# Jackson-D-Taylor/PINT

Hardware: AMD Instinct MI355X
Metric: GLS fits/sec, 68-PSR x 10k-TOA synthetic PTA (whole node) (higher is better)
Workload: dtype f64+dd; 1 GPU; pta68x10k GLSFitter.fit_toas(maxiter=1) incl. noise realisations (the 68-pulsar PTA, LPT-sharded over 1 rank(s)); npsr=68, ntoas=10000, K_cols_max=178, launch=direct, pipelines=2, parallelism=pulsar shards x1 (LPT, no data-path collective)

## Files before the change

include/pint_amd.h:

```cpp
#ifndef PINT_AMD_H
#define PINT_AMD_H

#include <stddef.h>
#include <stdint.h>

#ifdef __cplusplus
extern "C" {
#endif

#define PINT_OK 0
#define PINT_E_INVALID 1
#define PINT_E_HIP 2
#define PINT_E_NOT_PD 3
#define PINT_E_KEPLER 4
#define PINT_E_PARAM 5
#define PINT_E_SIGMA 6

#define PINT_MAX_COLS 320
#define PINT_MAX_F 16
#define PINT_MAX_DMK 10
#define PINT_MAX_FD 10
#define PINT_MAX_JUMP 64
#define PINT_MAX_GLITCH 64
#define PINT_MAX_WAVEX 128
// ... 100 lines not shown
    int32_t col_toff[PINT_MAX_COLS];
} pint_spec_t;

typedef struct pint_ctx pint_ctx;

pint_ctx *pint_ctx_create(int device);
void pint_ctx_destroy(pint_ctx *ctx);
const char *pint_last_error(pint_ctx *ctx);

void pint_release_cache(void);
int pint_device_count(void);
int pint_nslot(void);

int pint_add_pulsar(pint_ctx *ctx, const pint_toas_t *toas, const pint_spec_t *spec,
                    const double *red_freq, const double *red_phi);
int pint_add_pulsar_cols(pint_ctx *ctx, const pint_toa_cols_t *cols, const pint_spec_t *spec,
                         const double *red_freq, const double *red_phi);
int pint_set_wavex(pint_ctx *ctx, int psr, int o_wx, int nwx, int o_dmwx, int ndmwx);
int pint_set_chromatic(pint_ctx *ctx, int psr, int o_cm, int ncm, int o_cmwx, int ncmwx);

int pint_set_instances(pint_ctx *ctx, int ninst, const int32_t *inst_psr, const double *tables);

int pint_set_grid(pint_ctx *ctx, int psr, int npts, const double *base, int nvar, const int32_t *var_toff,
                  const int64_t *var_stride, const int64_t *var_size, const double *vals, int64_t k0);
int pint_get_tables(pint_ctx *ctx, double *tables_out);
int pint_set_tables(pint_ctx *ctx, const double *tables);

int pint_eval(pint_ctx *ctx, int want_M);

int pint_read_resids(pint_ctx *ctx, double *time_resid, double *phase_resid, double *chi2_wls);
int pint_read_eval(pint_ctx *ctx, double *phase_hi, double *phase_lo, double *ftaylor, double *delay);
int pint_read_designmatrix(pint_ctx *ctx, double *M);

int pint_fit_step(pint_ctx *ctx, int mode);
int pint_read_step(pint_ctx *ctx, double *dpars, double *errs, double *cov, double *chi2_lin);

int pint_apply_step(pint_ctx *ctx, const double *lambda_);
int pint_apply_step_uniform(pint_ctx *ctx, double lambda_);
int pint_fit_step_apply(pint_ctx *ctx, int mode, double lambda_);

int pint_save_tables(pint_ctx *ctx);
int pint_restore_tables(pint_ctx *ctx);

int pint_chi2_gls(pint_ctx *ctx, double *chi2);

int pint_chi2_wls(pint_ctx *ctx, double *chi2);

int pint_set_ecorr(pint_ctx *ctx, int psr, int nep, const int32_t *ep_ptr, const int32_t *ep_idx,
                   const double *ep_phi);

int pint_fit_layout(pint_ctx *ctx, int psr, int32_t *out4);
int pint_vgram_layout(pint_ctx *ctx, int psr, int32_t *out4);
int pint_set_wideband(pint_ctx *ctx, int psr, const double *pp_dm, const double *pp_dme,
                      const double *dm_sigma, const uint64_t *dmjump_mask);
int pint_dm_resids(pint_ctx *ctx, int subtract_mean, int use_weighted_mean, double *resid_out,
                   double *chi2_out);

int pint_set_lazy(pint_ctx *ctx, int lazy);
int pint_check(pint_ctx *ctx);

#ifndef PINT_NSLOT
#define PINT_NSLOT 4
#endif
int pint_step_end(pint_ctx *ctx, int *slot);
int pint_fit_step_enqueue(pint_ctx *ctx, int restore, int mode, double lambda_, double *dpars, double *errs,
                          double *cov, double *chi2lin, double *noise_red, double *noise_ecorr, double *noise_dm,
                          double *chi2, int *slot);
int pint_check_step(pint_ctx *ctx, int slot);
#define PINT_OPT_BLOCKED_SOLVE 1
#define PINT_OPT_VGRAM 2
#define PINT_OPT_TIMING_MASK 3
#define PINT_OPT_TIMING_EVERY 8
#define PINT_OPT_REFINE 4
#define PINT_OPT_VBIN 5
#define PINT_OPT_WBFIT 6
#define PINT_OPT_COV_DEFER 7
#define PINT_OPT_SCHUR 9
#define PINT_OPT_SMALL 10
#define PINT_OPT_LA_CHOL 11
#define PINT_OPT_EFUSE 12
#define PINT_OPT_LANE_SOLVE 13
#define PINT_OPT_SPIN_EVAL 14
#define PINT_OPT_SOLVE_W8 15
int pint_set_option(pint_ctx *ctx, int key, int value);
#define PINT_EIG_MAXDEG 8
int pint_solve_eig(pint_ctx *ctx, int mode, const double *threshold, int32_t *ndeg, double *degvec,
                   int degstride);

int pint_lognorm(pint_ctx *ctx, int gls, double *out);

int pint_capture_begin(pint_ctx *ctx);
int pint_capture_end(pint_ctx *ctx);
int pint_graph_launch(pint_ctx *ctx);
#define PINT_QUERY_NVGRAM 1
#define PINT_QUERY_NSPLIT 2
#define PINT_QUERY_NSPINEVAL 3
int pint_query(pint_ctx *ctx, int key);
void *pint_host_alloc(size_t bytes);
void pint_host_free(void *p);
int pint_debug_read(pint_ctx *ctx, int which, double *out);
int pint_debug_gram(pint_ctx *ctx, int pre_ecorr, double *out);
int pint_debug_set_resids(pint_ctx *ctx, const double *time_resid);

int pint_read_norms(pint_ctx *ctx, int mode, double *out);

int pint_inst_status(pint_ctx *ctx, int32_t *out);

int pint_noise_resids(pint_ctx *ctx, double *red, double *ecorr);
int pint_noise_resids_dm(pint_ctx *ctx, double *dm);

int pint_last_timing(pint_ctx *ctx, double *ms8);
int pint_sync(pint_ctx *ctx);

int pint_set_resids(pint_ctx *ctx, const double *time_resid);
int pint_set_sigma(pint_ctx *ctx, int psr, const double *sigma_s);
int pint_set_noise_weights(pint_ctx *ctx, int psr, const double *red_phi, const double *ep_phi);
int pint_set_noise_classes(pint_ctx *ctx, int psr, int ncls, const int32_t *cls_ptr, const int32_t *cls_idx,
                           const double *sigma0_us);
int pint_noise_lnlike(pint_ctx *ctx, const int32_t *kind, const double *cls_qf, const double *ep_w, double *out3,
                      double *cls_g, double *ep_g);

#ifdef __cplusplus
}
#endif
#endif
```

pint_amd/csrc/physics.hpp:

```cpp
#pragma once
#include "dd.hpp"
#include "../../include/pint_amd.h"

namespace pint {

constexpr double C_KMS = 299792.458;
constexpr double AU_KM = 149597870.7;
constexpr double KPC_KM = 3.0856775814913674e16;
constexpr double TSUN = 4.92549094830932e-06;
__device__ __constant__ const double TPLANET[5] = {TSUN / 1047.3486, TSUN / 3497.898, TSUN / 408523.71, TSUN / 22902.98,
                               TSUN / 19412.24};
constexpr double DMCONST = 4149.377593360996;
constexpr double DAYSEC = 86400.0;
constexpr double DJY = 365.25;
constexpr double ERFA_DC = 173.1446326742403;
constexpr double DR2AS = 206264.80624709636;
constexpr double MAS_RAD = 4.84813681109536e-09;
constexpr double HA_RAD = 0.2617993877991494;
constexpr double DEG_RAD = 0.017453292519943295;
constexpr double MASYR_RADS = 1.5362818500441604e-16;
constexpr double YR_S = 31557600.0;
constexpr double TWO_PI = 6.283185307179586;
constexpr double PI_D = 3.141592653589793;
constexpr double INV_C_KMS = 1.0 / C_KMS;
constexpr double INV_AU_KM = 1.0 / AU_KM;
constexpr double INV_AUC = 1.0 / (AU_KM * C_KMS);
constexpr double INV_KPC_KM = 1.0 / KPC_KM;
constexpr double INV_DJY = 1.0 / DJY;
constexpr double INV_TWO_PI = 1.0 / TWO_PI;
constexpr int NINV = 64;
__device__ __constant__ const double INV_HI[NINV] = {0.0, 1.0, 0.5, 0.3333333333333333, 0.25, 0.2, 0.16666666666666666, 0.14285714285714285, 0.125, 0.1111111111111111, 0.1, 0.09090909090909091, 0.08333333333333333, 0.07692307692307693, 0.07142857142857142, 0.06666666666666667, 0.0625, 0.058823529411764705, 0.05555555555555555, 0.05263157894736842, 0.05, 0.047619047619047616, 0.045454545454545456, 0.043478260869565216, 0.041666666666666664, 0.04, 0.038461538461538464, 0.037037037037037035, 0.03571428571428571, 0.034482758620689655, 0.03333333333333333, 0.03225806451612903, 0.03125, 0.030303030303030304, 0.029411764705882353, 0.02857142857142857, 0.027777777777777776, 0.02702702702702703, 0.02631578947368421, 0.02564102564102564, 0.025, 0.024390243902439025, 0.023809523809523808, 0.023255813953488372, 0.022727272727272728, 0.022222222222222223, 0.021739130434782608, 0.02127659574468085, 0.020833333333333332, 0.02040816326530612, 0.02, 0.0196078431372549, 0.019230769230769232, 0.018867924528301886, 0.018518518518518517, 0.01818181818181818, 0.017857142857142856, 0.017543859649122806, 0.017241379310344827, 0.01694915254237288, 0.016666666666666666, 0.01639344262295082, 0.016129032258064516, 0.015873015873015872};
__device__ __constant__ const double INV_LO[NINV] = {0.0, 0.0, 0.0, 1.850371707708594e-17, 0.0, -1.1102230246251566e-17, 9.25185853854297e-18, 7.93016446160826e-18, 0.0, 6.1679056923619804e-18, -5.551115123125783e-18, -2.523234146875356e-18, 4.625929269271485e-18, -4.270088556250602e-18, 3.96508223080413e-18, 9.251858538542971e-19, 0.0, 8.163404592832033e-19, 3.0839528461809902e-18, 2.921639538487254e-18, -2.7755575615628915e-18, 2.64338815386942e-18, -1.261617073437678e-18, 1.206764157201257e-18, 2.3129646346357427e-18, -8.326672684688674e-19, -2.135044278125301e-18, 2.05596856412066e-18, 1.982541115402065e-18, 4.785444071660157e-19, 4.625929269271486e-19, 8.953411488912552e-19, 0.0, -8.410780489584519e-19, 4.0817022964160166e-19, 8.921435019309293e-19, 1.5419764230904951e-18, -1.50030138462859e-18, 1.460819769243627e-18, 8.896017825522087e-19, -1.3877787807814458e-18, -8.46206573647223e-19, 1.32169407693471e-18, 3.2273925134452225e-19, -6.30808536718839e-19, -8.480870326997723e-19, 6.033820786006285e-19, 5.167261417803255e-19, 1.1564823173178713e-18, 1.6285159162231251e-18, -4.163336342344337e-19, 2.7211348642773444e-19, -1.0675221390626506e-18, 7.20073895688486e-19, 1.02798428206033e-18, 8.831319514063744e-19, 9.912705577010326e-19, 9.73879846162418e-19, 2.3927220358300787e-19, 5.880418562633244e-20, 2.312964634635743e-19, -8.531426931033477e-19, 4.476705744456276e-19, 8.8112938462314e-19};
PD double inv_int(int k) { return k < NINV ? INV_HI[k] : 1.0 / (double)k; }
PD dd dd_div_int(dd a, int k) { return k < NINV ? dd_mul(a, dd_make(INV_HI[k], INV_LO[k])) : dd_div_d(a, (double)k); }

PD double pval(const double* P, int o) { return P[o] + P[o + 1]; }
PD dd pdd(const double* P, int o) { return dd_make(P[o], P[o + 1]); }

struct PmState {
    double p[3], v1[3], tl1;
};

struct PmTrig {
    double cra, sra, cdec, sdec, cra2, sra2, cdec2, sdec2;
};

PD void pm_setup_trig(double pmr, double pmd, double px, const PmTrig& T, PmState& st);

PD void pm_setup(double ra, double dec, double pmr, double pmd, double px, PmState& st) {
    const double ra2 = ra + pmr, dec2 = dec + pmd;
    const PmTrig T = {cos(ra), sin(ra), cos(dec), sin(dec), cos(ra2), sin(ra2), cos(dec2), sin(dec2)};
    pm_setup_trig(pmr, pmd, px, T, st);
}

PD void pm_setup_trig(double pmr, double pmd, double px, const PmTrig& T, PmState& st) {
    double a1[3] = {T.cra * T.cdec, T.sra * T.cdec, T.sdec};
    double b1[3] = {T.cra2 * T.cdec2, T.sra2 * T.cdec2, T.sdec2};
    double cx = a1[1] * b1[2] - a1[2] * b1[1];
    double cy = a1[2] * b1[0] - a1[0] * b1[2];
    double cz = a1[0] * b1[1] - a1[1] * b1[0];
    double ss = sqrt(cx * cx + cy * cy + cz * cz);
    double cs = a1[0] * b1[0] + a1[1] * b1[1] + a1[2] * b1[2];
    double px1a = px;
    if ((ss != 0.0 || cs != 0.0) && !(cs > 0.0 && 326.0 * (ss / cs) * (1.0 + 1e-12) < px1a)) {
        const double pm = 326.0 * atan2(ss, cs);
        if (px1a < pm) px1a = pm;
    }
    if (px1a < 5e-7) px1a = 5e-7;
    double w = px1a >= 1e-7 ? px1a : 1e-7;
    double r = DR2AS / w;
    double rad = pmr / DJY, decd = pmd / DJY;
    double st_ = T.sra, ct = T.cra, sp = T.sdec, cp = T.cdec;
    double rcp = r * cp;
    double x = rcp * ct, y = rcp * st_;
    double rpd = r * decd;
    double ww = rpd * sp;
    double p[3] = {x, y, r * sp};
    double v[3] = {-y * rad - ww * ct, x * rad - ww * st_, rpd * cp};
    double vm = sqrt(v[0] * v[0] + v[1] * v[1] + v[2] * v[2]);
    if (vm / ERFA_DC > 0.5) { v[0] = v[1] = v[2] = 0.0; }
    double pm_ = sqrt(p[0] * p[0] + p[1] * p[1] + p[2] * p[2]);
    double xu[3] = {p[0] / pm_, p[1] / pm_, p[2] / pm_};
    double vsr = xu[0] * v[0] + xu[1] * v[1] + xu[2] * v[2];
    double usr[3] = {vsr * xu[0], vsr * xu[1], vsr * xu[2]};
    double ust[3] = {v[0] - usr[0], v[1] - usr[1], v[2] - usr[2]};
    double vst = sqrt(ust[0] * ust[0] + ust[1] * ust[1] + ust[2] * ust[2]);
    double betsr = vsr / ERFA_DC, betst = vst / ERFA_DC;
    double bett = betst, betr = betsr, d = 1.0, del = 0.0, od = 0.0, odel = 0.0, odd = 0.0, oddel = 0.0;
    for (int i = 0; i < 100; i++) {
        d = 1.0 + betr;
        double w2 = betr * betr + bett * bett;
        del = -w2 / (sqrt(1.0 - w2) + 1.0);
        betr = d * betsr + del;
        bett = d * betst;
        if (i > 0) {
            double dd_ = fabs(d - od), ddel = fabs(del - odel);
            if (i > 1 && dd_ >= odd && ddel >= oddel) break;
            odd = dd_;
            oddel = ddel;
        }
        od = d;
        odel = del;
    }
    double wr = (betsr != 0.0) ? d + del / betsr : 1.0;
    for (int k = 0; k < 3; k++) {
        st.p[k] = p[k];
        st.v1[k] = wr * usr[k] + d * ust[k];
    }
    st.tl1 = pm_ / ERFA_DC;
}

PD void pm_dir(const PmState& st, double dt_days, double out[3]) {
    const double* p = st.p;
    const double* v1 = st.v1;
    const double tl1 = st.tl1;
    double q[3] = {p[0] + (dt_days + tl1) * v1[0], p[1] + (dt_days + tl1) * v1[1], p[2] + (dt_days + tl1) * v1[2]};
    double r2 = q[0] * q[0] + q[1] * q[1] + q[2] * q[2];
// ... 765 lines not shown
}

PD double bt_deriv(const BinState& B, int pid) {
    const double e = B.ecc, sE = B.sinE, cE = B.cosE, tt0 = B.tt0, a1 = B.a1;
    const double sw = B.sw, cw = B.cw, sq = B.sqE, iom = B.iomeE;
    const double iP = B.iPBs, iP2 = iP * iP;
    const double dL1_dE = -a1 * sw * sE;
    const double dL2_dE = (a1 * cw * sq + B.GAMMA) * cE;
    const double dE_dECC = sE * iom;
    double dL1 = 0.0, dL2 = 0.0, dE = 0.0;
    switch (pid) {
        case PINT_B_A1: case PINT_B_A1DOT: {
            const double f = (pid == PINT_B_A1DOT) ? tt0 : 1.0;
            dL1 = f * sw * (cE - e);
            dL2 = f * cw * sq * sE;
        } break;
        case PINT_B_OM: case PINT_B_OMDOT: {
            const double f = (pid == PINT_B_OMDOT) ? tt0 : 1.0;
            dL1 = f * a1 * cw * (cE - e);
            dL2 = -f * a1 * sw * sq * sE;
        } break;
        case PINT_B_ECC: case PINT_B_EDOT: {
            const double f = (pid == PINT_B_EDOT) ? tt0 : 1.0;
            dL1 = f * (a1 * sw + dL1_dE * dE_dECC);
            dL2 = f * (-a1 * cw * e * sE / sq + dL2_dE * dE_dECC);
        } break;
        case PINT_B_GAMMA: dL2 = sE; break;
        case PINT_B_T0:
            dE = (((B.PBDOT - B.XPBDOT) * tt0 * iP - 1.0) * TWO_PI * iP - B.EDOT * sE) * iom;
            break;
        case PINT_B_PB: dE = TWO_PI * ((B.PBDOT + B.XPBDOT) * tt0 * tt0 * iP2 * iP - tt0 * iP2) * iom; break;
        case PINT_B_PBDOT: case PINT_B_XPBDOT: dE = -PI_D * tt0 * tt0 * iP2 * iom; break;
        default: break;
    }
    if (dE != 0.0) {
        dL1 = dL1_dE * dE;
        dL2 = dL2_dE * dE;
    }
    return B.R0 * (dL1 + dL2);
}

struct ToaRow {
    dd tdb;
    double freq;
    double pos[3], vel[3], sun[3];
    const double* planet;
    uint32_t flags;
    uint64_t jmask;
    int dmx_a, dmx_b;
    const int32_t* dmx_x;
    int dmx_x0, dmx_x1;
};

struct EvalOut {
    dd phase;
    double delay;
    double fdt;
    double ftaylor;
    double dmc;
    double inv_f2;
    int status;
};

PD dd spin_phase(const pint_spec_t& S, const double* P, dd dt) {
    int m = S.nf;
    dd r = pdd(P, S.o_F + 2 * (m - 1));
    for (int j = m - 1; j >= 1; j--) {
        r = dd_add(dd_div_int(dd_mul(r, dt), j + 1), pdd(P, S.o_F + 2 * (j - 1)));
    }
    return dd_mul(r, dt);
}
PD double spin_freq(const pint_spec_t& S, const double* P, double dt) {
    int m = S.nf;
    double r = pval(P, S.o_F + 2 * (m - 1));
    for (int j = m - 1; j >= 1; j--) r = r * dt * inv_int(j) + pval(P, S.o_F + 2 * (j - 1));
    return r;
}

struct ColRun {
    int kind, col0, cnt, idx0;
    int dcol0;
    int pad_[3];
};

struct EvalHead {
    double delay;
    double gLON, gLAT, gPMLON, gPMLAT, gPX;
    double inv_f2, dt_yr_dm, logf;
    double swg;
};
constexpr int EVAL_HEAD_W = 10;

struct EvalSpin {
    dd dt;
    double dtd, chain;
};
PD void eval_spin_a(const pint_spec_t& S, const double* P, const InstConst& C, const ToaRow& t, double delay,
                    EvalOut& o, EvalSpin& sp) {
    o.delay = delay;
    dd dt0 = dd_mul_d(dd_sub(t.tdb, pdd(P, S.o_PEPOCH)), DAYSEC);
    sp.dt = dd_add_d(dt0, -delay);
    sp.dtd = dd_to_d(sp.dt);
    o.fdt = spin_freq(S, P, sp.dtd);
    o.ftaylor = spin_freq(S, P, dd_to_d(dt0));
    sp.chain = o.fdt * C.iF0;
}

PD double glitch_dt(const pint_spec_t& S, const double* P, dd tdb, double delay, int k) {
    const int o = S.o_GLITCH + 2 * PINT_GL_NPAR * k;
    return dd_to_d(dd_add_d(dd_mul_d(dd_sub(tdb, pdd(P, o + 2 * PINT_GL_EP)), DAYSEC), -delay));
}
PD double glitch_phase_at(const double* G, double dt) {
    double ph = pval(G, 2 * PINT_GL_PH) +
                dt * (pval(G, 2 * PINT_GL_F0) +
                      dt * (0.5 * pval(G, 2 * PINT_GL_F1) + dt * ((1.0 / 6.0) * pval(G, 2 * PINT_GL_F2))));
    const double f0d = pval(G, 2 * PINT_GL_F0D);
    if (f0d != 0.0) {
        const double tau = pval(G, 2 * PINT_GL_TD) * DAYSEC;
        ph += f0d * tau * (1.0 - exp(-dt / tau));
    }
    return ph;
}
PD double glitch_col_at(const double* G, int which, double dt, double iF0) {
    const double tau = pval(G, 2 * PINT_GL_TD) * DAYSEC;
    const double f0d = pval(G, 2 * PINT_GL_F0D);
    const double e = tau != 0.0 ? exp(-dt / tau) : 0.0;
    double d;
    switch (which) {
        case PINT_GL_PH: d = 1.0; break;
        case PINT_GL_F0: d = dt; break;
        case PINT_GL_F1: d = 0.5 * dt * dt; break;
        case PINT_GL_F2: d = (1.0 / 6.0) * dt * dt * dt; break;
        case PINT_GL_F0D: d = tau * (1.0 - e); break;
        case PINT_GL_TD:
            d = tau != 0.0 ? (f0d * (1.0 - e) - f0d * e * (dt / tau)) * DAYSEC : 0.0;
            break;
        default:
            d = -(pval(G, 2 * PINT_GL_F0) +
                  dt * (pval(G, 2 * PINT_GL_F1) + 0.5 * dt * pval(G, 2 * PINT_GL_F2)) + f0d * e) * DAYSEC;
    }
    return -d * iF0;
}

PD dd glitch_row_phase(const pint_spec_t& S, const double* P, dd tdb, double delay, dd ph) {
    for (int k = 0; k < S.nglitch; k++) {
        const double gdt = glitch_dt(S, P, tdb, delay, k);
        if (gdt > 0.0) ph = dd_add_d(ph, glitch_phase_at(P + S.o_GLITCH + 2 * PINT_GL_NPAR * k, gdt));
    }
    return ph;
}
PD void glitch_row_columns(const pint_spec_t& S, const double* P, dd tdb, double delay, double iF0, double* Mb,
                           unsigned r, long ld, const ColRun* runs, int nrun, bool compact) {
    for (int u = 0; u < nrun; u++) {
        const ColRun R = runs[u];
        if (R.kind != PINT_COL_GLITCH) continue;
        double* colp = Mb + (long)(compact ? R.dcol0 : R.col0) * ld;
        for (int j = 0; j < R.cnt; j++, colp += ld) {
            const int k = (R.idx0 + j) / PINT_GL_NPAR, which = (R.idx0 + j) - PINT_GL_NPAR * k;
            const double gdt = glitch_dt(S, P, tdb, delay, k);
            colp[r] = gdt > 0.0 ? glitch_col_at(P + S.o_GLITCH + 2 * PINT_GL_NPAR * k, which, gdt, iF0) : 0.0;
        }
    }
}

template <int BIN>
PD void eval_spin_b(const pint_spec_t& S, const double* P, const InstConst& C, const ToaRow& t, const EvalHead& h,
                    const EvalSpin& sp, EvalOut& o, double* Mb, unsigned r, long ld, const ColRun* runs, int nrun,
                    bool compact, const double* swg = nullptr) {
    const double chain = sp.chain, dtd = sp.dtd;
    dd ph = spin_phase(S, P, sp.dt);
    if (S.njump > 0 && t.jmask) {
        dd F0 = pdd(P, S.o_F);
        for (int k = 0; k < S.njump; k++)
            if ((t.jmask >> k) & 1ull) ph = dd_add(ph, dd_mul(dd_make(pval(P, S.o_JUMP + 2 * k)), F0));
    }
    if (S.o_PHOFF >= 0 && r < (unsigned)ld) ph = dd_sub(ph, pdd(P, S.o_PHOFF));
    o.phase = ph;
    if (!Mb) return;
    const double iF0 = C.iF0;
    const double dt_yr_dm = h.dt_yr_dm, logf = h.logf;
    const double gLON = h.gLON * chain;
    const double gLAT = h.gLAT * chain;
    const double gPMLON = h.gPMLON * chain;
    const double gPMLAT = h.gPMLAT * chain;
    const double gPX = h.gPX * chain;
    const double dmc = chain * DMCONST * h.inv_f2;
    o.dmc = dmc;
    for (int u = 0; u < nrun; u++) {
        const ColRun R = runs[u];
        if (compact && R.kind == PINT_COL_DMX) continue;
        double* colp = Mb + (long)(compact ? R.dcol0 : R.col0) * ld;
        switch (R.kind) {
            case PINT_COL_OFFSET: colp[r] = iF0; break;
            case PINT_COL_F: {
                double v = 1.0;
                for (int j = 1; j <= R.idx0; j++) v = v * dtd * inv_int(j);
                for (int j = 0; j < R.cnt; j++, colp += ld) {
                    v = v * dtd * inv_int(R.idx0 + j + 1);
                    colp[r] = -v * iF0;
                }
            } break;
            case PINT_COL_JUMP:
                for (int j = 0; j < R.cnt; j++, colp += ld) colp[r] = ((t.jmask >> (R.idx0 + j)) & 1ull) ? -1.0 : 0.0;
                break;
            case PINT_COL_LON: colp[r] = gLON; break;
            case PINT_COL_LAT: colp[r] = gLAT; break;
            case PINT_COL_PMLON: colp[r] = gPMLON; break;
            case PINT_COL_PMLAT: colp[r] = gPMLAT; break;
            case PINT_COL_PX: colp[r] = gPX; break;
            case PINT_COL_DM: {
                double v = 1.0;
                for (int j = 1; j <= R.idx0; j++) v = v * dt_yr_dm * inv_int(j);
                for (int j = 0; j < R.cnt; j++, colp += ld) {
                    if (j > 0) v = v * dt_yr_dm * inv_int(R.idx0 + j);
                    colp[r] = dmc * v;
                }
            } break;
            case PINT_COL_NESW: {
                double g = h.swg;
                if (swg) {
                    unsigned rr = r;
                    asm volatile("" : "+v"(rr));
                    g = swg[rr];
                }
                colp[r] = h.inv_f2 > 1.0 ? 0.0 : dmc * g;
            } break;
            case PINT_COL_DMX:
                for (int j = 0; j < R.cnt; j++, colp += ld) {
                    const int idx = R.idx0 + j;
                    bool in = t.dmx_a == idx || t.dmx_b == idx;
                    for (int k = t.dmx_x0; k < t.dmx_x1; k++) in |= t.dmx_x[k] == idx;
                    colp[r] = in ? dmc : 0.0;
                }
                break;
            case PINT_COL_FD: {
                double v = 1.0;
                for (int j = 0; j <= R.idx0; j++) v *= logf;
                for (int j = 0; j < R.cnt; j++, colp += ld) {
                    if (j > 0) v *= logf;
                    colp[r] = chain * v;
                }
            } break;
            case PINT_COL_BIN:
                if (BIN == 0)
                    for (int j = 0; j < R.cnt; j++, colp += ld) colp[r] = 0.0;
                break;
            default:
                for (int j = 0; j < R.cnt; j++, colp += ld) colp[r] = 0.0;
        }
    }
}

struct EvalPre {
    EvalHead h;
    double fd;
    double L[3];
};
PD void eval_pre(const pint_spec_t& S, const double* P, const InstConst& C, const ToaRow& t, EvalOut& o, bool wantM,
                 EvalPre& pre, const double* swg, unsigned r) {
    o.status = 0;
    o.dmc = 0.0;
    double delay = 0.0;
    double L[3] = {0, 0, 1};
    double tdb_f = dd_to_d(t.tdb);
    bool has_pos = (t.flags & 2u) != 0;
    bool is_bary = (t.flags & 1u) != 0;
    double rr = 0.0, re_dot_L = 0.0;
    double px_mas = S.o_px >= 0 ? pval(P, S.o_px) : 0.0;
    if (S.astrometry) {
        psr_dir_icrs(C, tdb_f, L);
        rr = t.pos[0] * t.pos[0] + t.pos[1] * t.pos[1] + t.pos[2] * t.pos[2];
        re_dot_L = t.pos[0] * L[0] + t.pos[1] * L[1] + t.pos[2] * L[2];
        if (has_pos) {
            double d = -re_dot_L * INV_C_KMS;
            if (px_mas != 0.0) {
                d += (0.5 * (rr * px_mas * INV_KPC_KM) * (1.0 - re_dot_L * re_dot_L / rr)) * INV_C_KMS;
            }
            delay += d;
        }
    }
    if (S.shapiro && !is_bary) {
        double rs = sqrt(t.sun[0] * t.sun[0] + t.sun[1] * t.sun[1] + t.sun[2] * t.sun[2]);
        double rct = t.sun[0] * L[0] + t.sun[1] * L[1] + t.sun[2] * L[2];
        double ds = -2.0 * TSUN * log((rs - rct) * INV_AU_KM);
        if (S.shapiro == 2) {
#pragma unroll 1
            for (int q = 0; q < 5; q++) {
                const double x = t.planet[3 * q], y = t.planet[3 * q + 1], z = t.planet[3 * q + 2];
                const double rp = sqrt(x * x + y * y + z * z);
                const double rcp = x * L[0] + y * L[1] + z * L[2];
                ds += -2.0 * TPLANET[q] * log((rp - rcp) * INV_AU_KM);
            }
        }
        delay += ds;
    }
    double bfreq = t.freq;
    if (S.astrometry) {
        double vdl = t.vel[0] * L[0] + t.vel[1] * L[1] + t.vel[2] * L[2];
        bfreq = t.freq * (1.0 - vdl * INV_C_KMS);
    }
    double inv_f2 = 1.0 / (bfreq * bfreq);
    o.inv_f2 = inv_f2;
    if (S.o_NE_SW >= 0) delay += (pval(P, S.o_NE_SW) * swg[r]) * DMCONST * inv_f2;
    double dt_yr_dm = 0.0;
    if (S.ndm > 0) {
        bool any = false;
        for (int k = 1; k < S.ndm; k++) any |= (pval(P, S.o_DM + 2 * k) != 0.0);
        if (S.o_DMEPOCH >= 0) {
            dd dtd = dd_sub(t.tdb, pdd(P, S.o_DMEPOCH));
            dt_yr_dm = dd_to_d(dtd) * INV_DJY;
        }
        double x = any ? dt_yr_dm : 0.0;
        double dm = pval(P, S.o_DM + 2 * (S.ndm - 1));
        for (int k = S.ndm - 1; k >= 1; k--) dm = dm * x * inv_int(k) + pval(P, S.o_DM + 2 * (k - 1));
        delay += dm * DMCONST * inv_f2;
    }
    if (S.ndmx > 0) {
        double dmx = 0.0;
        if (t.dmx_a >= 0) dmx += pval(P, S.o_DMX + 2 * t.dmx_a);
        if (t.dmx_b >= 0) dmx += pval(P, S.o_DMX + 2 * t.dmx_b);
        for (int k = t.dmx_x0; k < t.dmx_x1; k++) dmx += pval(P, S.o_DMX + 2 * t.dmx_x[k]);
        delay += dmx * DMCONST * inv_f2;
    }
    double logf = 0.0;
    double fd = 0.0;
    if (S.nfd > 0) {
        logf = log(bfreq * 1e-3);
        if (!isfinite(logf)) logf = 0.0;
        for (int k = S.nfd; k >= 1; k--) fd = fd * logf + pval(P, S.o_FD + 2 * (k - 1));
        fd *= logf;
    }
    double gLON = 0, gLAT = 0, gPMLON = 0, gPMLAT = 0, gPX = 0;
    if (wantM && S.astrometry) {
        double u[3] = {t.pos[0], t.pos[1], t.pos[2]};
        if (S.astrometry == 2) {
            double ue[3] = {u[0], u[1], u[2]};
            icrs_to_ecl(S.obliquity, ue, u);
        }
        const double r_km = sqrt(rr);
        const double ir = r_km > 0.0 ? 1.0 / r_km : 0.0;
        const double ced_sdl = (C.splon * u[0] - C.cplon * u[1]) * ir;
        const double ced_cdl = (C.cplon * u[0] + C.splon * u[1]) * ir;
        const double sed = u[2] * ir;
        const double te_s = S.o_POSEPOCH >= 0 ? dd_to_d(dd_mul_d(dd_sub(t.tdb, pdd(P, S.o_POSEPOCH)), DAYSEC)) : 0.0;
        const double rc = r_km * INV_C_KMS;
        gLON = rc * (ced_sdl * C.cplat) * (S.astrometry == 1 ? HA_RAD : DEG_RAD);
        gLAT = rc * (ced_cdl * C.splat - sed * C.cplat) * DEG_RAD;
        gPMLON = rc * ced_sdl * te_s * MASYR_RADS;
        gPMLAT = rc * (ced_cdl * C.splat - C.cplat * sed) * te_s * MASYR_RADS;
        gPX = 0.5 * ((rr - re_dot_L * re_dot_L) * INV_AUC) * MAS_RAD;
    }
    pre.h = {delay, gLON, gLAT, gPMLON, gPMLAT, gPX, inv_f2, dt_yr_dm, logf, 0.0};
    pre.fd = fd;
    pre.L[0] = L[0];
    pre.L[1] = L[1];
    pre.L[2] = L[2];
}

PD void eval_head(const pint_spec_t& S, const double* P, const InstConst& C, const ToaRow& t, EvalHead& h,
                  const double* swg, unsigned r) {
    EvalOut o;
    EvalPre pre;
    eval_pre(S, P, C, t, o, true, pre, swg, r);
    h = pre.h;
    if (S.o_NE_SW >= 0) h.swg = swg[r];
    if (S.nfd > 0) h.delay += pre.fd;
}

template <int BIN>
PD void eval_toa(const pint_spec_t& S, const double* P, const InstConst& C, const ToaRow& t, EvalOut& o,
                 double* Mb, unsigned r, long ld, const ColRun* runs, int nrun, bool compact, const double* swg) {
    EvalPre pre;
    eval_pre(S, P, C, t, o, Mb != nullptr, pre, swg, r);
    double delay = pre.h.delay;
    const double* L = pre.L;
    const double fd = pre.fd;
    const double inv_f2 = pre.h.inv_f2, dt_yr_dm = pre.h.dt_yr_dm, logf = pre.h.logf;
    const double gLON = pre.h.gLON, gLAT = pre.h.gLAT, gPMLON = pre.h.gPMLON, gPMLAT = pre.h.gPMLAT, gPX = pre.h.gPX;
    BinState B;
    B.status = 0;
    if (BIN == 1 || BIN == 3) {
        ell1_setup<BIN == 3>(S, P, C, t.tdb, delay, B);
        delay += B.delay;
    } else if (BIN == 2) {
        ddm_setup(S, P, C, t.tdb, delay, B);
        delay += B.delay;
        if (B.status) o.status = B.status;
    } else if (BIN == 4) {
        bt_setup(S, P, C, t.tdb, delay, B);
        delay += B.delay;
        if (B.status) o.status = B.status;
    } else if (BIN == 5) {
        double ko[3] = {t.pos[0], t.pos[1], t.pos[2]}, kp[3] = {L[0], L[1], L[2]};
        if (S.astrometry == 2) {
            icrs_to_ecl(S.obliquity, t.pos, ko);
            icrs_to_ecl(S.obliquity, L, kp);
        }
        ddm_setup<true>(S, P, C, t.tdb, delay, B, ko, kp);
        delay += B.delay;
        if (B.status) o.status = B.status;
    }
    if (S.nfd > 0) delay += fd;
    EvalSpin sp;
    eval_spin_a(S, P, C, t, delay, o, sp);
    const double chain = sp.chain;
    if (Mb && BIN != 0) {
        Ell1Grad eg;
        if (BIN == 1 || BIN == 3) ell1_grad<BIN == 3>(B, eg);
        for (int u = 0; u < nrun; u++) {
            const ColRun R = runs[u];
            if (R.kind != PINT_COL_BIN) continue;
            double* colp = Mb + (long)(compact ? R.dcol0 : R.col0) * ld;
            for (int j = 0; j < R.cnt; j++, colp += ld) {
                const int pid = S.col_index[R.col0 + j];
                double d = 0.0;
                if (BIN == 1 || BIN == 3) d = ell1_deriv(B, eg, pid);
                if (BIN == 2) d = ddm_deriv(B, pid);
                if (BIN == 4) d = bt_deriv(B, pid);
                if (BIN == 5) d = ddm_deriv<true>(B, pid);
                colp[r] = chain * d * bin_unit_factor(pid);
            }
        }
    }
    const EvalHead h = {delay, gLON, gLAT, gPMLON, gPMLAT, gPX, inv_f2, dt_yr_dm, logf, 0.0};
    eval_spin_b<BIN>(S, P, C, t, h, sp, o, Mb, r, ld, runs, nrun, compact, S.o_NE_SW >= 0 ? swg : nullptr);
}

}
```

pint_amd/csrc/pint_hip.hip:

```cpp
#include <hip/hip_runtime.h>
#include <hip/hip_ext.h>
#include <string>
#include <vector>
#include <cstring>
#include <cstdio>
#include <algorithm>
#include <cmath>
#include <cstdlib>
#include <map>
#include <type_traits>
#include <mutex>
#include <functional>
#include <chrono>
#include "physics.hpp"

using namespace pint;

typedef double double4_t __attribute__((ext_vector_type(4)));

__device__ __forceinline__ void rot(double& c, double& s, double c1, double s1) {
    const double cn = c * c1 - s * s1;
    s = s * c1 + c * s1;
    c = cn;
}
// ... 254 lines not shown
    __shared__ InstConst sC;
    inst_setup_wave(*reinterpret_cast<const pint_spec_t*>(sS), staged ? sP : Pg, sC, sx, threadIdx.x);
    __syncthreads();
    if (threadIdx.x == 0) *out = sC;
}

constexpr int PREP_LANE_TAB = 64;
__global__ __launch_bounds__(64) void k_prep_lanes(const PsrDev* __restrict__ psrs, const InstDev* __restrict__ insts,
                                                   int ninst, double* __restrict__ tables,
                                                   const double* __restrict__ tables0, InstConst* __restrict__ ic) {
    const int q = blockIdx.x * 64 + threadIdx.x;
    if (q >= ninst) return;
    const InstDev I = insts[q];
    const pint_spec_t& S = *psrs[I.psr].spec;
    const double* P = tables + I.toff;
    if (tables0) {
        const int ts = S.tstride;
        for (int i = 0; i < ts; i++) tables[I.toff + i] = tables0[I.toff + i];
        P = tables0 + I.toff;
    }
    InstConst C;
    inst_setup_seq(S, P, C);
    ic[q] = C;
}
__global__ __launch_bounds__(64) void k_apply_lanes(const PsrDev* __restrict__ psrs, const InstDev* __restrict__ insts,
                                                    int ninst, double* __restrict__ tables,
                                                    const double* __restrict__ dpars, const double* __restrict__ lam,
                                                    InstConst* __restrict__ ic, double lam_u) {
    const int q = blockIdx.x * 64 + threadIdx.x;
    if (q >= ninst) return;
    const InstDev I = insts[q];
    const pint_spec_t& S = *psrs[I.psr].spec;
    double* P = tables + I.toff;
    const double li = lam ? lam[q] : lam_u;
    if (li != 0.0) {
        for (int c = 0; c < S.ncol; c++) {
            const int o = S.col_toff[c];
            if (o < 0) continue;
            const dd v = dd_add_d(dd_make(P[o], P[o + 1]), li * dpars[I.coff + c]);
            P[o] = v.hi;
            P[o + 1] = v.lo;
        }
    }
    InstConst C;
    inst_setup_seq(S, P, C);
    ic[q] = C;
}

__global__ __launch_bounds__(PREP_T) void k_prep(const PsrDev* __restrict__ psrs, const InstDev* __restrict__ insts,
                                                 double* __restrict__ tables, const double* __restrict__ tables0,
                                                 InstConst* __restrict__ ic) {
    const InstDev I = insts[blockIdx.x];
    const PsrDev& Pd = psrs[I.psr];
    const int ts = Pd.spec->tstride;
    if (tables0) {
        for (int i = threadIdx.x; i < ts; i += PREP_T) tables[I.toff + i] = tables0[I.toff + i];
        prep_one(Pd.spec, tables0 + I.toff, ts, ic + blockIdx.x);
        return;
    }
    prep_one(Pd.spec, tables + I.toff, ts, ic + blockIdx.x);
}

constexpr int EVAL_MAXTAB = 512;
constexpr int EVAL_MAXRUN = 64;
struct alignas(16) EvalLds {
    pint_spec_t S;
    InstConst C;
    ColRun R[EVAL_MAXRUN];
    double P[EVAL_MAXTAB];
    double X[4];
    double red[8];
};
constexpr int EF_ROWS = 254;

struct EvalRestore {
    double* tables;
    InstConst* ic;
    double* rph;
    double* epart;
    const double* swg;
};

__device__ __forceinline__ void load_toa_row(const PsrDev& Pd, const pint_spec_t& S, unsigned r, ToaRow& t) {
    t.tdb = dd_make(Pd.tdb_hi[r], Pd.tdb_lo[r]);
    t.freq = Pd.freq[r];
#pragma unroll
    for (int k = 0; k < 3; k++) {
        t.pos[k] = Pd.pos[3 * r + k];
        t.vel[k] = Pd.vel[3 * r + k];
        t.sun[k] = Pd.sun[3 * r + k];
    }
    t.planet = S.shapiro == 2 ? Pd.planet + 15 * r : nullptr;
    t.flags = Pd.flags[r];
    t.jmask = Pd.jmask[r];
    t.dmx_a = Pd.dmx_a[r];
    t.dmx_b = Pd.dmx_b[r];
    t.dmx_x = Pd.dmx_x;
    t.dmx_x0 = Pd.dmx_x ? Pd.dmx_x[r] : 0;
    t.dmx_x1 = Pd.dmx_x ? Pd.dmx_x[r + 1] : 0;
}

template <int WANT_M, int BIN>
__device__ __forceinline__ void eval_row(const pint_spec_t& S, EvalLds& L, const PsrDev& Pd, const InstDev& I, bool stP,
                                         bool stR, int nrun, const double* __restrict__ tables, unsigned r, int n,
                                         bool own, double* __restrict__ Mout, double* __restrict__ dmxv, int compact,
                                         int write_red, int* __restrict__ status, int* __restrict__ istatus, int ii,
                                         double* __restrict__ ph_hi, double* __restrict__ ph_lo,
                                         double* __restrict__ ftay, double* __restrict__ delay_out,
                                         double* __restrict__ dfac, const double* __restrict__ swg, EvalOut& o) {
    const double* P = stP ? L.P : tables + I.toff;
    ToaRow t;
    load_toa_row(Pd, S, r, t);
    double* Mb = WANT_M ? (Mout + I.moff) : nullptr;
    const bool rowM = WANT_M && own && r < (unsigned)n;
    const bool cmp = WANT_M && compact && Pd.dsplit;
    eval_toa<BIN>(S, P, L.C, t, o, rowM ? Mb : nullptr, r, n, stR ? L.R : Pd.runs, nrun, cmp, swg ? swg + I.roff : nullptr);
    if (!own) return;
    if (rowM && cmp) dmxv[I.ooff + r] = o.dmc;
    if (o.status) {
        atomicOr(status, 1 << o.status);
        atomicOr(istatus + ii, 1 << o.status);
    }
    ph_hi[I.roff + r] = o.phase.hi;
    ph_lo[I.roff + r] = o.phase.lo;
    ftay[I.roff + r] = o.ftaylor;
    delay_out[I.roff + r] = o.delay;
    const bool dmn = S.dmn0 < S.nred;
    const double Dfac = 1400.0 * 1400.0 * o.inv_f2;
    if (WANT_M && rowM && dmn) dfac[I.ooff + r] = Dfac;
    if (WANT_M && rowM && S.nred > 0 && (write_red || dmn) && !(cmp && Pd.vg)) {
        dd ts = dd_mul_d(t.tdb, DAYSEC);
        double* colp = Mb + (long)(cmp ? Pd.red0c : S.ncol) * n;
        for (int k = write_red ? 0 : S.dmn0; k < S.nred; k++) {
            dd x = dd_mul(ts, dd_make(Pd.red_freq[k], Pd.red_freq[S.nred + k]));
            double fr = dd_to_d(dd_sub(x, dd_floor(x)));
            double sn, cs;
            sincos(TWO_PI * fr, &sn, &cs);
            const double sc = k >= S.dmn0 ? Dfac : 1.0;
            colp[2L * k * n + r] = sn * sc;
            colp[2L * k * n + r + n] = cs * sc;
        }
    }
}

template <int WANT_M, int BIN>
__device__ __forceinline__ void eval_block(int b, const PsrDev* __restrict__ psrs, const InstDev* __restrict__ insts,
                                           const int* __restrict__ blk_inst, const int* __restrict__ blk_row0,
                                           const double* __restrict__ tables, const InstConst* __restrict__ ic,
                                           double* __restrict__ ph_hi, double* __restrict__ ph_lo,
                                           double* __restrict__ ftay, double* __restrict__ delay_out,
                                           double* __restrict__ Mout, double* __restrict__ dmxv, int compact,
                                           int write_red, int* __restrict__ status, int* __restrict__ istatus,
                                           double* __restrict__ dfac, EvalLds& L, EvalRestore rs) {
    int ii = blk_inst[b];
    const InstDev I = insts[ii];
    const PsrDev& Pd = psrs[I.psr];
    const int ts = I.ts, nrun = I.nrun;
    const bool stP = ts <= EVAL_MAXTAB, stR = nrun <= EVAL_MAXRUN;
    {
        static_assert(sizeof(pint_spec_t) % 16 == 0 && sizeof(InstConst) % 16 == 0 && sizeof(ColRun) % 16 == 0,
                      "eval staging: 16-byte words");
        constexpr int NS = (int)(sizeof(pint_spec_t) / 16), NC = (int)(sizeof(InstConst) / 16);
        constexpr int RW = (int)(sizeof(ColRun) / 16);
        static_assert(NS <= 512 && NC + EVAL_MAXRUN * RW <= 256 && EVAL_MAXTAB <= 512, "eval staging: two rounds of 256");
        const int t = threadIdx.x;
        const int NR = stR ? nrun * RW : 0;
        const uint4* sg = reinterpret_cast<const uint4*>(I.spec);
        const uint4* cg = reinterpret_cast<const uint4*>(ic + ii);
        const uint4* rg = reinterpret_cast<const uint4*>(I.runs);
        const double* pg = tables + I.toff;
        const bool hs0 = t < NS, hs1 = t + 256 < NS, hc = t < NC, hr = !hc && t < NC + NR;
        const bool hp0 = stP && t < ts, hp1 = stP && t + 256 < ts;
        uint4 s0 = {}, s1 = {}, cr = {};
        double p0 = 0.0, p1 = 0.0;
        if (hs0) s0 = sg[t];
        if (hs1) s1 = sg[t + 256];
        if (hc) cr = cg[t];
        else if (hr) cr = rg[t - NC];
        if (hp0) p0 = pg[t];
        if (hp1) p1 = pg[t + 256];
        uint4* sd = reinterpret_cast<uint4*>(&L.S);
        if (hs0) sd[t] = s0;
        if (hs1) sd[t + 256] = s1;
        if (hc) reinterpret_cast<uint4*>(&L.C)[t] = cr;
        else if (hr) reinterpret_cast<uint4*>(L.R)[t - NC] = cr;
        if (hp0) L.P[t] = p0;
        if (hp1) L.P[t + 256] = p1;
    }
    __syncthreads();
    wgp_stamp(0, true);
    if (rs.tables && blk_row0[b] == 0) {
        for (int k = threadIdx.x; k < ts; k += blockDim.x) rs.tables[I.toff + k] = stP ? L.P[k] : tables[I.toff + k];
        const int* cs = reinterpret_cast<const int*>(&L.C);
        int* cd = reinterpret_cast<int*>(rs.ic + ii);
        for (int k = threadIdx.x; k < (int)(sizeof(InstConst) / 4); k += blockDim.x) cd[k] = cs[k];
    }
    const pint_spec_t& S = L.S;
    const int n = I.n;
    const bool ef = rs.epart != nullptr;
    const int lt = threadIdx.x;
    unsigned r;
    bool own;
    if (ef) {
        r = lt < EF_ROWS ? (unsigned)(blk_row0[b] + lt) : (lt == EF_ROWS ? 0u : (unsigned)n);
        own = lt < EF_ROWS ? r < (unsigned)n : (lt == EF_ROWS + 1 && blk_row0[b] == 0);
        if (lt < EF_ROWS && r >= (unsigned)n) r = 0;
    } else {
        r = (unsigned)(blk_row0[b] + lt);
        own = r <= (unsigned)n;
        if (!own) return;
    }
    EvalOut o;
    eval_row<WANT_M, BIN>(S, L, Pd, I, stP, stR, nrun, tables, r, n, own, Mout, dmxv, compact, write_red, status, istatus,
                          ii, ph_hi, ph_lo, ftay, delay_out, dfac, rs.swg, o);
    wgp_stamp(1, false);
    if (!ef) return;
    if (lt == EF_ROWS) {
        L.X[2] = o.phase.hi;
        L.X[3] = o.phase.lo;
    } else if (lt == EF_ROWS + 1) {
        L.X[0] = o.phase.hi;
        L.X[1] = o.phase.lo;
    }
    __syncthreads();
    const dd tz = dd_make(L.X[0], L.X[1]);
    dd d0 = dd_make(0.0);
    if (!S.track_pn && S.subtract_mean) d0 = dd_add_d(dd_sub(dd_make(L.X[2], L.X[3]), tz), Pd.dpn[0]);
    double sw = 0.0, swx = 0.0;
    if (lt < EF_ROWS && own) {
        const dd d = dd_add_d(dd_sub(dd_make(o.phase.hi, o.phase.lo), tz), Pd.dpn[r]);
        double full;
        if (S.track_pn) {
            full = dd_to_d(dd_add_d(d, -Pd.pn[r]));
        } else {
            const dd x = dd_sub(d, d0);
            full = dd_to_d(dd_sub(x, dd_round_half_up(x)));
        }
        rs.rph[I.roff - ii + r] = full;
        const double lw = Pd.isig[r];
        const double w = S.weighted_mean ? lw * lw : 1.0;
        sw += w;
        swx += w * full;
    }
    if (S.subtract_mean) {
        double v[2] = {swx, sw};
        block_sums<4, 2>(v, L.red);
        if (lt == 0) {
            const long eb = I.eb0 + blk_row0[b] / EF_ROWS;
            rs.epart[2 * eb] = v[1];
            rs.epart[2 * eb + 1] = v[0];
        }
    }
}

__device__ __forceinline__ double sw_geometry_row(const PsrDev& Pd, const InstConst& C, int i) {
    double L[3];
    psr_dir_icrs(C, dd_to_d(dd_make(Pd.tdb_hi[i], Pd.tdb_lo[i])), L);
    const double sun[3] = {Pd.sun[3 * i], Pd.sun[3 * i + 1], Pd.sun[3 * i + 2]};
    return solar_wind_geometry_pc(sun, L);
}
__global__ __launch_bounds__(256) void k_sw_geom(const PsrDev* __restrict__ psrs, const InstDev* __restrict__ insts,
                                                 const InstConst* __restrict__ ic, double* __restrict__ swg) {
    const InstDev I = insts[blockIdx.x];
    const PsrDev& Pd = psrs[I.psr];
    if (Pd.spec->o_NE_SW < 0) return;
    const int r = blockIdx.y * 256 + threadIdx.x;
    if (r > I.n) return;
    swg[I.roff + r] = sw_geometry_row(Pd, ic[blockIdx.x], r);
}

template <bool ROT>
__device__ __forceinline__ double wavex_harmonic(const double* H, dd dt_days, double shift, double& s, double& c) {
    const double f2 = 2.0 * pval(H, 0);
    const dd x = dd_mul_d(dt_days, f2);
    const double n = 2.0 * rint(0.5 * x.hi);
    sincospi((x.hi - n) + x.lo, &s, &c);
    double sa = s, ca = c;
    if (ROT) {
        const double e = PI_D * f2 * shift, e2 = e * e;
        double se, ce;
        if (fabs(e) <= 0.0625) {
            se = e * (1.0 - e2 * (1.0 / 6.0) * (1.0 - e2 * (1.0 / 20.0) * (1.0 - e2 * (1.0 / 42.0))));
            ce = 1.0 - e2 * 0.5 * (1.0 - e2 * (1.0 / 12.0) * (1.0 - e2 * (1.0 / 30.0) * (1.0 - e2 * (1.0 / 56.0))));
        } else {
            sincos(e, &se, &ce);
        }
        sa = s * ce - c * se;
        ca = c * ce + s * se;
    }
    return pval(H, 2) * sa + pval(H, 4) * ca;
}
template <bool ROT>
__device__ __forceinline__ double wavex_component(const double* B, int nh, dd dt_days, double shift, int kind,
                                                  double scale, double* Mb, bool wr, unsigned r, long ld,
                                                  const ColRun* runs, int nrun, bool compact) {
    int u0 = 0, u1 = 0;
    if (Mb) {
        u0 = nrun;
        for (int u = 0; u < nrun; u++)
            if (runs[u].kind == kind) {
                u0 = u < u0 ? u : u0;
                u1 = u + 1;
            }
    }
    double v = 0.0;
    for (int k = 0; k < nh; k++) {
        double s, c;
        v += wavex_harmonic<ROT>(B + 6 * k, dt_days, shift, s, c);
        for (int u = u0; u < u1; u++) {
            const ColRun R = runs[u];
            if (R.kind != kind) continue;
            const long col = compact ? R.dcol0 : R.col0;
            const int js = 2 * k - R.idx0, jc = js + 1;
            if (wr && js >= 0 && js < R.cnt) Mb[(col + js) * ld + r] = scale * s;
            if (wr && jc >= 0 && jc < R.cnt) Mb[(col + jc) * ld + r] = scale * c;
        }
    }
    return v;
}
template <bool CHROM>
__global__ __launch_bounds__(256) void k_wavex(const PsrDev* __restrict__ psrs, const InstDev* __restrict__ insts,
                                               const double* __restrict__ tables, const InstConst* __restrict__ ic,
// ... 69 lines not shown
        }
    }
    delay[I.roff + r] = tot;
    dd ph = dd_sub(dd_make(ph_hi[I.roff + r], ph_lo[I.roff + r]), two_prod(dsum, fdt));
    if (CHROM && ncm + ncmwx > 0) {
        double f1 = 0.0;
        if (S.nf > 1) {
            f1 = pval(P, S.o_F + 2 * (S.nf - 1));
            for (int j = S.nf - 2; j >= 1; j--) f1 = f1 * dtd * inv_int(j) + pval(P, S.o_F + 2 * j);
        }
        ph = dd_add_d(ph, 0.5 * dsum * dsum * f1);
        if (!(fabs(dsum) <= PINT_MAX_ADDED_DELAY)) {
            atomicOr(status, 1 << PINT_E_PARAM);
            atomicOr(istatus + blockIdx.x, 1 << PINT_E_PARAM);
        }
    }
    ph_hi[I.roff + r] = ph.hi;
    ph_lo[I.roff + r] = ph.lo;
}

__global__ __launch_bounds__(256) void k_glitch(const PsrDev* __restrict__ psrs, const InstDev* __restrict__ insts,
                                                const double* __restrict__ tables, const InstConst* __restrict__ ic,
                                                const double* __restrict__ delay, double* __restrict__ ph_hi,
                                                double* __restrict__ ph_lo, double* __restrict__ Mout, int compact) {
    const InstDev I = insts[blockIdx.x];
    const PsrDev& Pd = psrs[I.psr];
    const pint_spec_t& S = *Pd.spec;
    if (S.nglitch <= 0) return;
    const int r = blockIdx.y * 256 + threadIdx.x;
    if (r > I.n) return;
    const double* P = tables + I.toff;
    const dd tdb = dd_make(Pd.tdb_hi[r], Pd.tdb_lo[r]);
    const double dl = delay[I.roff + r];
    const dd ph = glitch_row_phase(S, P, tdb, dl, dd_make(ph_hi[I.roff + r], ph_lo[I.roff + r]));
    ph_hi[I.roff + r] = ph.hi;
    ph_lo[I.roff + r] = ph.lo;
    if (Mout && r < I.n)
        glitch_row_columns(S, P, tdb, dl, ic[blockIdx.x].iF0, Mout + I.moff, (unsigned)r, I.n, Pd.runs, Pd.nrun,
                           compact && Pd.dsplit);
}

__global__ __launch_bounds__(256) void k_eval_head(const PsrDev* __restrict__ psrs, const InstDev* __restrict__ insts,
                                                   const double* __restrict__ tables, const InstConst* __restrict__ ic,
                                                   const double* __restrict__ swg, double* __restrict__ shr) {
    const InstDev I = insts[0];
    const PsrDev& Pd = psrs[I.psr];
    const pint_spec_t& S = *Pd.spec;
    const unsigned r = blockIdx.x * 256 + threadIdx.x;
    if (r > (unsigned)I.n) return;
    ToaRow t;
    load_toa_row(Pd, S, r, t);
    EvalHead h;
    eval_head(S, tables + I.toff, ic[0], t, h, swg ? swg + I.roff : nullptr, r);
    double* o = shr + (long)r * EVAL_HEAD_W;
    o[0] = h.delay;
    o[1] = h.gLON;
    o[2] = h.gLAT;
    o[3] = h.gPMLON;
    o[4] = h.gPMLAT;
    o[5] = h.gPX;
    o[6] = h.inv_f2;
    o[7] = h.dt_yr_dm;
    o[8] = h.logf;
    o[9] = h.swg;
}

__global__ __launch_bounds__(256) void k_eval_spin(const PsrDev* __restrict__ psrs, const InstDev* __restrict__ insts,
                                                   int ninst, const double* __restrict__ tables,
                                                   const InstConst* __restrict__ ic, const double* __restrict__ shr,
                                                   double* __restrict__ ph_hi, double* __restrict__ ph_lo,
                                                   double* __restrict__ ftay, double* __restrict__ delay_out,
                                                   double* __restrict__ Mout) {
    const int ii = blockIdx.x * 4 + (int)__builtin_amdgcn_readfirstlane(threadIdx.x >> 6);
    if (ii >= ninst) return;
    const InstDev I = insts[ii];
    const PsrDev& Pd = psrs[I.psr];
    const pint_spec_t& S = *Pd.spec;
    const InstConst C = ic[ii];
    const double* P = tables + I.toff;
    const int n = I.n;
    double* Mb = Mout + I.moff;
    for (int r = threadIdx.x & 63; r <= n; r += 64) {
        ToaRow t;
        t.tdb = dd_make(Pd.tdb_hi[r], Pd.tdb_lo[r]);
        t.jmask = Pd.jmask[r];
        t.dmx_a = Pd.dmx_a[r];
        t.dmx_b = Pd.dmx_b[r];
        t.dmx_x = Pd.dmx_x;
        t.dmx_x0 = Pd.dmx_x ? Pd.dmx_x[r] : 0;
        t.dmx_x1 = Pd.dmx_x ? Pd.dmx_x[r + 1] : 0;
        const double* q = shr + (long)r * EVAL_HEAD_W;
        const EvalHead h = {q[0], q[1], q[2], q[3], q[4], q[5], q[6], q[7], q[8], q[9]};
        EvalOut o;
        o.status = 0;
        o.dmc = 0.0;
        o.inv_f2 = h.inv_f2;
        EvalSpin sp;
        eval_spin_a(S, P, C, t, h.delay, o, sp);
        eval_spin_b<0>(S, P, C, t, h, sp, o, r < n ? Mb : nullptr, (unsigned)r, n, Pd.runs, Pd.nrun, false);
        ph_hi[I.roff + r] = o.phase.hi;
        ph_lo[I.roff + r] = o.phase.lo;
        ftay[I.roff + r] = o.ftaylor;
        delay_out[I.roff + r] = o.delay;
    }
}

template <int WANT_M, int BIN, int W = 0>
__global__ __launch_bounds__(256) __attribute__((amdgpu_waves_per_eu(W > 0 ? W : 1, W > 0 ? W : 10)))
void k_eval(const PsrDev* __restrict__ psrs, const InstDev* __restrict__ insts,
                                              const int* __restrict__ blk_inst, const int* __restrict__ blk_row0,
                                              const double* __restrict__ tables, const InstConst* __restrict__ ic,
                                              double* __restrict__ ph_hi, double* __restrict__ ph_lo,
                                              double* __restrict__ ftay, double* __restrict__ delay_out,
                                              double* __restrict__ Mout, double* __restrict__ dmxv, int compact,
                                              int write_red, int* __restrict__ status, int* __restrict__ istatus,
                                              double* __restrict__ dfac, EvalRestore rs) {
    __shared__ EvalLds L;
    eval_block<WANT_M, BIN>(blockIdx.x, psrs, insts, blk_inst, blk_row0, tables, ic, ph_hi, ph_lo, ftay, delay_out,
                            Mout, dmxv, compact, write_red, status, istatus, dfac, L, rs);
}

template <int WANT_M>
__device__ __forceinline__ void eval_mix_body(const PsrDev* __restrict__ psrs, const InstDev* __restrict__ insts,
                                                  const int* __restrict__ blk_inst, const int* __restrict__ blk_row0,
                                                  int off1, int off2, int off3,
                                                  const double* __restrict__ tables, const InstConst* __restrict__ ic,
                                                  double* __restrict__ ph_hi, double* __restrict__ ph_lo,
                                                  double* __restrict__ ftay, double* __restrict__ delay_out,
                                                  double* __restrict__ Mout, double* __restrict__ dmxv, int compact,
                                                  int write_red, int* __restrict__ status, int* __restrict__ istatus,
                                                  double* __restrict__ dfac, EvalRestore rs) {
    const int n2 = off3 - off2, n1 = off2 - off1;
    const int b = blockIdx.x;
    __shared__ EvalLds L;
    if (b < n2)
        eval_block<WANT_M, 2>(off2 + b, psrs, insts, blk_inst, blk_row0, tables, ic, ph_hi, ph_lo, ftay, delay_out,
                              Mout, dmxv, compact, write_red, status, istatus, dfac, L, rs);
    else if (b < n2 + n1)
        eval_block<WANT_M, 1>(off1 + b - n2, psrs, insts, blk_inst, blk_row0, tables, ic, ph_hi, ph_lo, ftay,
                              delay_out, Mout, dmxv, compact, write_red, status, istatus, dfac, L, rs);
    else
        eval_block<WANT_M, 0>(b - n2 - n1, psrs, insts, blk_inst, blk_row0, tables, ic, ph_hi, ph_lo, ftay, delay_out,
                              Mout, dmxv, compact, write_red, status, istatus, dfac, L, rs);
}
#define PINT_EVAL_MIX_ARGS                                                                                      \
    const PsrDev *__restrict__ psrs, const InstDev *__restrict__ insts, const int *__restrict__ blk_inst,        \
        const int *__restrict__ blk_row0, int off1, int off2, int off3, const double *__restrict__ tables,      \
        const InstConst *__restrict__ ic, double *__restrict__ ph_hi, double *__restrict__ ph_lo,               \
        double *__restrict__ ftay, double *__restrict__ delay_out, double *__restrict__ Mout,                   \
        double *__restrict__ dmxv, int compact, int write_red, int *__restrict__ status,                        \
        int *__restrict__ istatus, double *__restrict__ dfac, EvalRestore rs
#define PINT_EVAL_MIX_PASS                                                                                      \
    psrs, insts, blk_inst, blk_row0, off1, off2, off3, tables, ic, ph_hi, ph_lo, ftay, delay_out, Mout, dmxv,  \
        compact, write_red, status, istatus, dfac, rs
template <int WANT_M>
__global__ __launch_bounds__(256) void k_eval_mix(PINT_EVAL_MIX_ARGS) {
    WgTimer wgt_(WGT_EVAL);
    eval_mix_body<WANT_M>(PINT_EVAL_MIX_PASS);
}
template <int WANT_M, int W>
__global__ __launch_bounds__(256) __attribute__((amdgpu_waves_per_eu(W, W))) void k_eval_mix_w(PINT_EVAL_MIX_ARGS) {
    WgTimer wgt_(WGT_EVAL);
    eval_mix_body<WANT_M>(PINT_EVAL_MIX_PASS);
}

constexpr int RES_BT = 256;
constexpr int RES_RB = 1024;
constexpr int RES_RPT = RES_RB / RES_BT;
constexpr int RES_SMALLN = 64 * RES_RPT;
template <int BT>
__global__ __launch_bounds__(RES_BT) void k_resid1(const PsrDev* __restrict__ psrs, const InstDev* __restrict__ insts,
                                                   const int* __restrict__ rblk_inst, int nrblk,
                                                   const double* __restrict__ ph_hi, const double* __restrict__ ph_lo,
                                                   double* __restrict__ rphase, double* __restrict__ rpart) {
    WgTimer wgt_(WGT_RES1);
    constexpr int NW = BT / 64;
    __shared__ double sh[2 * (RES_BT / 64)];
    const int rb = blockIdx.x * (RES_BT / BT) + (BT == RES_BT ? 0 : (int)__builtin_amdgcn_readfirstlane(threadIdx.x / BT));
    if (BT != RES_BT && rb >= nrblk) return;
    const int tid = threadIdx.x % BT;
    const int ii = rblk_inst[rb];
    const InstDev I = insts[ii];
    const PsrDev& Pd = psrs[I.psr];
    const pint_spec_t& S = *Pd.spec;
    const int n = I.n;
    const long ro = I.roff;
    const long oo = I.roff - ii;
    const int r0 = (int)(rb - I.rb0) * RES_RB;
    const int r1 = min(n, r0 + RES_RB);
    const dd tz = dd_make(ph_hi[ro + n], ph_lo[ro + n]);
    dd d0 = dd_make(0.0);
    if (!S.track_pn && S.subtract_mean) d0 = dd_add_d(dd_sub(dd_make(ph_hi[ro], ph_lo[ro]), tz), Pd.dpn[0]);
    double sw = 0.0, swx = 0.0;
    double lh[RES_RPT], ll[RES_RPT], lp[RES_RPT], lpn[RES_RPT], lw[RES_RPT];
#pragma unroll
    for (int u = 0; u < RES_RPT; u++) {
        const int i = r0 + tid + u * BT;
        const bool in = i < r1;
        lh[u] = in ? ph_hi[ro + i] : 0.0;
        ll[u] = in ? ph_lo[ro + i] : 0.0;
        lp[u] = in ? Pd.dpn[i] : 0.0;
        lpn[u] = (in && S.track_pn) ? Pd.pn[i] : 0.0;
        lw[u] = (in && S.weighted_mean) ? Pd.isig[i] : 1.0;
    }
#pragma unroll
    for (int u = 0; u < RES_RPT; u++) {
        const int i = r0 + tid + u * BT;
        if (i >= r1) break;
        dd d = dd_add_d(dd_sub(dd_make(lh[u], ll[u]), tz), lp[u]);
        double full;
        if (S.track_pn) {
            full = dd_to_d(dd_add_d(d, -lpn[u]));
        } else {
            dd x = dd_sub(d, d0);
            full = dd_to_d(dd_sub(x, dd_round_half_up(x)));
        }
        rphase[oo + i] = full;
        double w = S.weighted_mean ? lw[u] * lw[u] : 1.0;
        sw += w;
        swx += w * full;
    }
    if (S.subtract_mean) {
        double v[2] = {swx, sw};
        block_sums<NW, 2>(v, sh);
        swx = v[0];
        sw = v[1];
        if (tid == 0) {
            rpart[3 * rb] = sw;
            rpart[3 * rb + 1] = swx;
        }
    }
}

constexpr int WT_CS = 66;
constexpr int WT_CS2 = 34;
template <int BT>
__global__ __launch_bounds__(RES_BT) void k_resid2(const PsrDev* __restrict__ psrs, const InstDev* __restrict__ insts,
                                                   const int* __restrict__ rblk_inst, int nrblk,
                                                   const double* __restrict__ ftay,
                                                   double* __restrict__ rtime, double* __restrict__ rphase,
                                                   double* __restrict__ rpart, double* __restrict__ wtile,
                                                   const double* __restrict__ epart) {
    WgTimer wgt_(WGT_RES2);
    constexpr int NW = BT / 64;
    __shared__ double sh[2 * (RES_BT / 64)];
    extern __shared__ double xs[];
// ... 3970 lines not shown
    bool inflight[2] = {false, false};
    long flushes = 0;
    bool held = false;
    size_t cur_idx = (size_t)-1;
    PsrDev* cur_dev = nullptr;
    std::vector<void*> bufs;
    ~PendArena() { release(); }
    void release() {
        for (int k = 0; k < 2; k++) {
            if (done[k]) {
                if (inflight[k]) hipEventSynchronize(done[k]);
                hipEventDestroy(done[k]);
                done[k] = nullptr;
            }
            inflight[k] = false;
        }
        if (held) {
            std::lock_guard<std::mutex> lk(g_stage.mu);
            g_stage.busy = false;
            held = false;
        }
        host = nullptr;
        cap = 0;
        size = 0;
        fix.clear();
    }
};

struct PsrHost {
    PsrDev dev;
    pint_spec_t spec;
    std::vector<int> dlo, dhi;
    std::vector<int> drow_host;
    int dslot_ns = 0;
    std::vector<void*> bufs;
    int n, K;
    double f1 = 0.0, f1_lo = 0.0;
};

struct pint_ctx {
    int device = 0;
    hipStream_t stream = nullptr;
    hipStream_t cstream = nullptr;
    hipEvent_t ev_solved = nullptr, ev_copied = nullptr;
    hipStream_t sstream = nullptr;
    hipEvent_t ev_gram = nullptr, ev_sigma = nullptr;
    bool sigma_pending = false;
    std::string err;
    std::vector<PsrHost> psrs;
    std::vector<int> setup_pending;
    bool psrs_dirty = false;
    PsrDev* d_psrs = nullptr;
    int npsr_dev = 0;
    int ninst = 0;
    std::vector<InstDev> inst;
    InstDev* d_inst = nullptr;
    InstDev* d_inst_sorted = nullptr;
    InstDev* d_inst_sorted_c = nullptr;
    InstDev* d_inst_sorted_v = nullptr;
    bool sorted_alias[3] = {false, false, false};
    double* d_gridspec = nullptr;
    std::vector<KpGroup> kp_groups, kp_groups_c, kp_groups_v;
    int vgram = 1;
    int vbin = 1;
    int wbfit = 0;
    int gv_pair = 1;
    int maxn = 0;
    int max_ts = 0;
    int resid12 = 1;
    int prep_lanes = 1;
    int fuse_r2 = 1;
    bool r2_pending = false;
    bool grid_valid = false;
    std::vector<double> grid_spec_host;
    int grid_psr = -1;
    long grid_opts = 0;
    int small = 1;
    int schur = 1;
    int evalb_wpe = 3;
    int la_chol = 1;
    int solve_w8 = 1;
    int eval0_wpe = 1;
    int eval_wpe = 3;
    int n_vg = 0;
    bool any_dmx_rows = false;
    double *d_TSp = nullptr, *d_TS = nullptr;
    double* d_Sdp = nullptr;
    double* d_BFp = nullptr;
    int vb_on = 0;
    double* d_xw = nullptr;
    int cov_defer = 1;
    bool cov_pending = false;
    int cov_mode = 0;
    size_t cov_lds = 0;
    bool ic_valid = false;
    bool no_events = false;
    int timing_mask = 0xff;
    int timing_every = 1;
    long gram_calls = 0;
    static constexpr int NSLOT = PINT_NSLOT;
    hipGraph_t graph_s[NSLOT] = {};
    hipGraphExec_t graph_exec_s[NSLOT] = {};
    bool capturing = false;
    int* d_blk_inst = nullptr;
    int* d_blk_row0 = nullptr;
    int* d_rblk_inst = nullptr;
    double* d_rpart = nullptr;
    double* d_epart = nullptr;
    int efz = 0;
    bool any_glitch = false;
    bool any_wavex = false;
    bool any_chrom = false;
    int efuse = 1;
    int lane_solve = 1;
    std::vector<int> upsr;
    int spin_grid = 0;
    bool tables_fresh = false;
    int spin_eval = 1;
    int n_spin_eval = 0;
    double* d_shr = nullptr;
    long shr_cap = 0;
    int nrblk = 0;
    int eval_merge = 0;
    int nblk = 0;
    int blk_off[PINT_NBIN + 1] = {0};
    long tot_table = 0, tot_rows = 0, tot_m = 0, tot_g = 0, tot_s = 0, tot_c = 0, tot_out = 0, tot_cv = 0;
    int lazy = 0;
    int blocked_solve = 1;
    int refine = 1;
    int gvdbg = 0;
    int nsplit = 1;
    double *d_tables = nullptr, *d_phhi = nullptr, *d_phlo = nullptr, *d_ftay = nullptr, *d_delay = nullptr;
    double* d_swg = nullptr;
    double *d_M = nullptr, *d_rt = nullptr, *d_rp = nullptr, *d_chi2 = nullptr, *d_chi2lin = nullptr;
    double *d_G = nullptr, *d_colsq = nullptr, *d_work = nullptr, *d_dpars = nullptr, *d_errs = nullptr;
    double *d_cov = nullptr, *d_sigL = nullptr, *d_lam = nullptr, *d_chi2g = nullptr;
    double *d_esum = nullptr, *d_eD = nullptr, *d_eW = nullptr, *d_ecs = nullptr, *d_wpart = nullptr;
    double* d_eC = nullptr;
    double* d_lognorm = nullptr;
    double *d_eigw = nullptr, *d_degv = nullptr;
    int* d_ndeg = nullptr;
    size_t eig_cap = 0;
    int degv_cap = 0;
    InstConst* d_ic = nullptr;
    InstConst* d_ic0 = nullptr;
    bool apply_req = false;
    bool apply_done = false;
    double apply_lam = 1.0;
    bool ic0_valid = false;
    double *d_dmxv = nullptr, *d_Sd = nullptr, *d_DD = nullptr, *d_DCS = nullptr;
    double* d_dfac = nullptr;
    int max_ndc = 0;
    int m_compact = 0;
    int red_valid[2] = {0, 0};
    size_t wpart_cap = 0;
    double *d_dmr = nullptr, *d_dmc2 = nullptr;
    long dmr_cap = 0, dmc2_cap = 0;
    long tot_e = 0, tot_ep = 0;
    int max_nep = 0;
    int* d_status = nullptr;
    int* d_istatus = nullptr;
    double* d_rscr = nullptr;
    int maxK = 0;
    static constexpr int NEV = 16, NMS = 8;
    int slot = 0;
    hipEvent_t ev_slot[NSLOT][NEV] = {};
// ... 404 lines not shown
    for (auto& p : ctx->psrs) all.push_back(p.dev);
    HIPCHK(hipMalloc(&ctx->d_psrs, sizeof(PsrDev) * all.size()));
    HIPCHK(h2d(ctx->d_psrs, all.data(), sizeof(PsrDev) * all.size(), nullptr, true));
    return 0;
}

extern "C" {

int pint_nslot(void) { return pint_ctx::NSLOT; }

int pint_device_count(void) {
    int n = 0;
    if (hipGetDeviceCount(&n) != hipSuccess) return 0;
    return n;
}

static std::mutex g_stream_mu;
static std::map<int, std::map<long, hipStream_t>> g_stream_pool[3];
static std::map<hipStream_t, long> g_stream_rank;
static long g_stream_made = 0;
enum { STREAM_KERNEL = 0, STREAM_COPY = 1, STREAM_SIDE = 2 };
static int g_stream_pool_on = -1;
static bool stream_pool_on() {
    if (g_stream_pool_on < 0) g_stream_pool_on = getenv("PINT_STREAM_POOL") ? (atoi(getenv("PINT_STREAM_POOL")) != 0) : 1;
    return g_stream_pool_on != 0;
}
static hipStream_t stream_get(int device, int role) {
    std::lock_guard<std::mutex> lk(g_stream_mu);
    auto& v = g_stream_pool[role][device];
    if (stream_pool_on() && !v.empty()) {
        hipStream_t s = v.begin()->second;
        v.erase(v.begin());
        return s;
    }
    hipStream_t s = nullptr;
    if (hipStreamCreateWithFlags(&s, hipStreamNonBlocking) != hipSuccess) return nullptr;
    g_stream_rank[s] = g_stream_made++;
    return s;
}
static void stream_put(int device, int role, hipStream_t s) {
    if (!s) return;
    hipStreamSynchronize(s);
    if (!stream_pool_on()) {
        hipStreamDestroy(s);
        return;
    }
    std::lock_guard<std::mutex> lk(g_stream_mu);
    g_stream_pool[role][device][g_stream_rank[s]] = s;
}

pint_ctx* pint_ctx_create(int device) {
    pint_ctx* ctx = new pint_ctx();
    ctx->device = device;
    if (hipSetDevice(device) != hipSuccess) {
        ctx->err = "hipSetDevice failed";
        return ctx;
    }
    ctx->stream = stream_get(device, STREAM_KERNEL);
    ctx->cstream = stream_get(device, STREAM_COPY);
    const unsigned evf = hipEventDisableTiming |
                         ((getenv("PINT_EV_SYSTEM") && atoi(getenv("PINT_EV_SYSTEM"))) ? 0u : hipEventReleaseToDevice);
    hipEventCreateWithFlags(&ctx->ev_solved, evf);
    hipEventCreateWithFlags(&ctx->ev_copied, evf);
    hipEventCreateWithFlags(&ctx->ev_noise, evf);
    if (getenv("PINT_SERIAL") && atoi(getenv("PINT_SERIAL"))) ctx->sstream = ctx->stream;
    else ctx->sstream = stream_get(device, STREAM_SIDE);
    ctx->no_events = getenv("PINT_NO_EVENTS") && atoi(getenv("PINT_NO_EVENTS"));
    ctx->eval_merge = getenv("PINT_EVAL_MERGE") ? atoi(getenv("PINT_EVAL_MERGE")) : 3;
    ctx->vbin = getenv("PINT_VBIN") ? (atoi(getenv("PINT_VBIN")) ? 1 : 0) : 1;
    ctx->cov_defer = getenv("PINT_COV_DEFER") ? atoi(getenv("PINT_COV_DEFER")) : 1;
    ctx->eval_wpe = getenv("PINT_EVAL_WPE") ? atoi(getenv("PINT_EVAL_WPE")) : 3;
    ctx->gv_pair = getenv("PINT_GV_PAIR") ? atoi(getenv("PINT_GV_PAIR")) : 1;
    ctx->schur = getenv("PINT_SCHUR") ? atoi(getenv("PINT_SCHUR")) : 1;
    ctx->fuse_r2 = getenv("PINT_FUSE_R2") ? atoi(getenv("PINT_FUSE_R2")) : 1;
    ctx->eval0_wpe = getenv("PINT_EVAL0_WPE") ? atoi(getenv("PINT_EVAL0_WPE")) : 1;
    ctx->prep_lanes = getenv("PINT_PREP_LANES") ? atoi(getenv("PINT_PREP_LANES")) : 1;
    ctx->resid12 = getenv("PINT_RESID12") ? atoi(getenv("PINT_RESID12")) : 1;
    ctx->evalb_wpe = getenv("PINT_EVALB_WPE") ? atoi(getenv("PINT_EVALB_WPE")) : 3;
    ctx->la_chol = getenv("PINT_LA_CHOL") ? atoi(getenv("PINT_LA_CHOL")) : 1;
    ctx->solve_w8 = getenv("PINT_SOLVE_W8") ? atoi(getenv("PINT_SOLVE_W8")) : 1;
    ctx->efuse = getenv("PINT_EFUSE") ? atoi(getenv("PINT_EFUSE")) : 1;
    ctx->lane_solve = getenv("PINT_LANE_SOLVE") ? atoi(getenv("PINT_LANE_SOLVE")) : 1;
    ctx->spin_eval = getenv("PINT_SPIN_EVAL") ? atoi(getenv("PINT_SPIN_EVAL")) : 1;
    hipEventCreateWithFlags(&ctx->ev_gram, evf);
    hipEventCreateWithFlags(&ctx->ev_sigma, evf);
    for (int sl = 0; sl < pint_ctx::NSLOT; sl++) {
        hipEventCreateWithFlags(&ctx->ev_done[sl], evf);
        hipEventCreateWithFlags(&ctx->ev_cdone[sl], hipEventDisableTiming);
    }
    hipMalloc(&ctx->d_status_slots, pint_ctx::NSLOT * sizeof(int));
    hipMemset(ctx->d_status_slots, 0, pint_ctx::NSLOT * sizeof(int));
    ctx->d_status = ctx->d_status_slots;
    hipHostMalloc(&ctx->h_status, pint_ctx::NSLOT * sizeof(int), hipHostMallocDefault);
    if (ctx->h_status)
        for (int sl = 0; sl < pint_ctx::NSLOT; sl++) ctx->h_status[sl] = 0;
    return ctx;
}

const char* pint_last_error(pint_ctx* ctx) { return ctx ? ctx->err.c_str() : "null context"; }

static void free_instances(pint_ctx* ctx) {
    if (ctx->stream) hipStreamSynchronize(ctx->stream);
    if (ctx->cstream) hipStreamSynchronize(ctx->cstream);
    if (ctx->sstream) hipStreamSynchronize(ctx->sstream);
    InstDev** sorted[3] = {&ctx->d_inst_sorted, &ctx->d_inst_sorted_c, &ctx->d_inst_sorted_v};
    for (int l = 0; l < 3; l++) {
        if (ctx->sorted_alias[l]) *sorted[l] = nullptr;
        ctx->sorted_alias[l] = false;
    }
    dfree((void*&)ctx->d_gridspec);
    dfree((void*&)ctx->d_shr);
    ctx->shr_cap = 0;
    ctx->spin_grid = 0;
    for (int sl = 0; sl < pint_ctx::NSLOT; sl++) {
        void** pss[] = {(void**)&ctx->d_chi2lin_s[sl], (void**)&ctx->d_dpars_s[sl], (void**)&ctx->d_errs_s[sl],
                        (void**)&ctx->d_cov_s[sl], (void**)&ctx->d_chi2g_s[sl], (void**)&ctx->d_xw_s[sl]};
        for (auto p : pss) dfree(*p);
    }
    void** ps[] = {(void**)&ctx->d_inst, (void**)&ctx->d_inst_sorted, (void**)&ctx->d_blk_inst, (void**)&ctx->d_blk_row0, (void**)&ctx->d_tables,
                   (void**)&ctx->d_phhi, (void**)&ctx->d_phlo, (void**)&ctx->d_ftay, (void**)&ctx->d_delay, (void**)&ctx->d_swg,
                   (void**)&ctx->d_M, (void**)&ctx->d_rt, (void**)&ctx->d_rp, (void**)&ctx->d_chi2, (void**)&ctx->d_istatus, (void**)&ctx->d_rscr,
                   (void**)&ctx->d_G, (void**)&ctx->d_colsq,
                   (void**)&ctx->d_work, (void**)&ctx->d_sigL,
                   (void**)&ctx->d_lam, (void**)&ctx->d_lognorm,
                   (void**)&ctx->d_eigw,
                   (void**)&ctx->d_degv, (void**)&ctx->d_ndeg, (void**)&ctx->d_esum, (void**)&ctx->d_eD,
                   (void**)&ctx->d_eW, (void**)&ctx->d_eC, (void**)&ctx->d_ecs, (void**)&ctx->d_wpart, (void**)&ctx->d_ic, (void**)&ctx->d_ic0,
                   (void**)&ctx->d_dmxv, (void**)&ctx->d_Sd, (void**)&ctx->d_DD, (void**)&ctx->d_DCS,
                   (void**)&ctx->d_dfac, (void**)&ctx->d_inst_sorted_c, (void**)&ctx->d_inst_sorted_v, (void**)&ctx->d_Sdp,
                   (void**)&ctx->d_BFp, (void**)&ctx->d_TSp, (void**)&ctx->d_TS, (void**)&ctx->d_rblk_inst, (void**)&ctx->d_rpart, (void**)&ctx->d_epart,
                   (void**)&ctx->d_noise, (void**)&ctx->d_tables0,
                   (void**)&ctx->d_wtile, (void**)&ctx->d_norms, (void**)&ctx->d_ones};
    for (auto p : ps) dfree(*p);
    ctx->d_dpars = ctx->d_errs = ctx->d_cov = ctx->d_chi2lin = ctx->d_xw = ctx->d_chi2g = nullptr;
    clear_copy_pend(ctx);
    ctx->noise_cap = 0;
    ctx->tables0_cap = 0;
    ctx->ic0_valid = false;
    ctx->restore_pending = false;
    ctx->wfuse = ctx->wtile_valid = false;
    for (int k = 0; k < pint_ctx::NSLOT; k++) {
        if (ctx->graph_exec_s[k]) hipGraphExecDestroy(ctx->graph_exec_s[k]);
        if (ctx->graph_s[k]) hipGraphDestroy(ctx->graph_s[k]);
        ctx->graph_exec_s[k] = nullptr;
        ctx->graph_s[k] = nullptr;
    }
    ctx->ninst = 0;
    ctx->wpart_cap = 0;
    ctx->eig_cap = 0;
    ctx->degv_cap = 0;
}

void pint_ctx_destroy(pint_ctx* ctx) {
    if (!ctx) return;
    hipSetDevice(ctx->device);
    ctx->cq.clear();
    hipStreamSynchronize(ctx->stream);
    free_instances(ctx);
    ctx->pend.release();
    for (auto b : ctx->pend.bufs) hipFree(b);
    for (auto& p : ctx->psrs) {
        for (auto b : p.bufs) hipFree(b);
    }
    if (ctx->d_psrs) hipFree(ctx->d_psrs);
    if (ctx->d_dmr) hipFree(ctx->d_dmr);
    if (ctx->d_dmc2) hipFree(ctx->d_dmc2);
// ... 758 lines not shown
        I.n = ph.n;
        I.spec = ph.dev.spec;
        I.runs = ph.dev.runs;
        I.ts = ph.spec.tstride;
        I.nrun = ph.dev.nrun;
        I.K = ph.K;
        I.Kp = ph.dev.Kp;
        I.toff = toff;
        I.roff = roff;
        I.moff = moff;
        I.goff = goff;
        I.soff = soff;
        I.coff = coff;
        I.cvoff = cvoff;
        I.eoff = eoff;
        I.epoff = epoff;
        I.ooff = out;
        I.sdoff = sdoff;
        I.ddoff = ddoff;
        I.vgoff = vgoff;
        I.vboff = vboff;
        I.xwoff = xwoff;
        if (ph.dev.vg) {
            vgoff += (long)nsplit * ph.dev.vns * (ph.dev.Kd + 3);
            if (ph.dev.vb) vboff += (long)nsplit * GW * ph.dev.vns * 128;
            ctx->n_vg++;
        } else if (ph.dev.dsplit) {
            ctx->any_dmx_rows = true;
        }
        if (ph.dev.dsplit) {
            sdoff += (long)ph.dev.ndc * ph.dev.Kpd;
            ddoff += ph.dev.ndc;
            const long nbd = (ph.dev.Kd + 15) / 16, nbk = (ph.dev.ndc + 15) / 16;
            xwoff += (nbd * (nbd + 1) / 2 + nbd * nbk) * 256 + (nbd + 3 * nbk) * 16 + schur_xw_extra(nbd, nbk);
            if (ph.dev.ndc > max_ndc) max_ndc = ph.dev.ndc;
        }
        I.self = k;
        I.rb0 = (long)rbi.size();
        I.nrb = std::max(1, (ph.n + RES_RB - 1) / RES_RB);
        for (int b = 0; b < I.nrb; b++) rbi.push_back(k);
        eoff += (long)ph.dev.nep * I.Kp;
        epoff += ph.dev.nep;
        if (ph.dev.nep > max_nep) max_nep = ph.dev.nep;
        cvoff += (long)ph.spec.ncol * ph.spec.ncol;
        toff += ph.spec.tstride;
        int bt = ph.spec.binary;
        if (bt < 0 || bt >= PINT_NBIN) { ctx->err = "bad binary model"; return PINT_E_INVALID; }
        if (ctx->efz) {
            I.eb0 = ebn;
            I.neb = std::max(1, (ph.n + EF_ROWS - 1) / EF_ROWS);
            ebn += I.neb;
            for (int r0 = 0; r0 < std::max(1, ph.n); r0 += EF_ROWS) {
                bti[bt].push_back(k);
                btr[bt].push_back(r0);
            }
        } else {
            I.eb0 = 0;
            I.neb = 0;
            for (int r0 = 0; r0 <= ph.n; r0 += 256) {
                bti[bt].push_back(k);
                btr[bt].push_back(r0);
            }
        }
        roff += ph.n + 1;
        moff += (long)ph.n * ph.K;
        goff += (long)(nsplit + 1) * I.Kp * I.Kp;
        soff += (long)(ph.K + 1) * (ph.K + 1);
        coff += ph.K + 1;
        out += ph.n;
        if (ph.K > maxK) maxK = ph.K;
    }
    ctx->ninst = ninst;
    ctx->tot_table = toff;
    ctx->tot_rows = roff;
    ctx->tot_m = moff;
    ctx->tot_g = goff;
    ctx->tot_s = soff;
    ctx->tot_c = coff;
    ctx->tot_out = out;
    ctx->tot_cv = cvoff;
    ctx->maxK = maxK;
    ctx->maxn = 0;
    ctx->max_ts = 0;
    for (const InstDev& I : ctx->inst) {
        ctx->maxn = std::max(ctx->maxn, I.n);
        ctx->max_ts = std::max(ctx->max_ts, ctx->psrs[I.psr].spec.tstride);
    }
    {
        std::vector<char> seen(ctx->psrs.size(), 0);
        ctx->upsr.clear();
        for (int k = 0; k < ninst; k++)
            if (!seen[inst_psr[k]]) {
                seen[inst_psr[k]] = 1;
                ctx->upsr.push_back(inst_psr[k]);
            }
    }
    ctx->tot_e = eoff;
    ctx->tot_ep = epoff;
    ctx->max_nep = max_nep;
    ctx->max_ndc = max_ndc;
    std::vector<int> bi, br;
    for (int t = 0; t < PINT_NBIN; t++) {
        ctx->blk_off[t] = (int)bi.size();
        bi.insert(bi.end(), bti[t].begin(), bti[t].end());
        br.insert(br.end(), btr[t].begin(), btr[t].end());
    }
    ctx->blk_off[PINT_NBIN] = (int)bi.size();
    ctx->nblk = ctx->blk_off[3];
    HIPCHK(cmalloc((void**)&ctx->d_inst, sizeof(InstDev) * ninst));
    HIPCHK(h2d(ctx->d_inst, ctx->inst.data(), sizeof(InstDev) * ninst, nullptr, true));
    for (int lay = 0; lay < 3; lay++) {
        std::vector<InstDev> sorted;
        std::vector<KpGroup>& groups = lay == 0 ? ctx->kp_groups : (lay == 1 ? ctx->kp_groups_c : ctx->kp_groups_v);
        groups.clear();
        const int maxT = lay == 2 ? 29 : GMAXT_ALL;
        std::vector<std::vector<int>> bucket(maxT + 1);
        std::vector<int> bkp(maxT + 1, 16);
        for (int k = 0; k < ninst; k++) {
            const InstDev& I = ctx->inst[k];
            const PsrDev& pd = ctx->psrs[I.psr].dev;
            if (lay == 1 && pd.dsplit && pd.vg) continue;
            if (lay == 2 && !(pd.dsplit && pd.vg)) continue;
            const int kp = lay == 2 ? pd.vkp : ((lay && pd.dsplit) ? pd.Kpd : I.Kp);
            const int nt = kp / 16;
            int tT = (nt * (nt + 1) / 2 + GWAVES - 1) / GWAVES;
            if (lay == 2) {
                const int ntr = (pd.red0c + 1 + pd.vns) / 16;
                tT = 10 * (ntr - 1) + nt;
            }
            if (lay < 2 && ctx->small && kp <= 32 && I.n <= GS_MAXN) tT = 0;
            if (tT < (lay < 2 ? 0 : 1) || tT > maxT) continue;
            bucket[tT].push_back(k);
            if (kp > bkp[tT]) bkp[tT] = kp;
        }
        if (lay == 2) {
            auto cost = [&](int k) {
                const PsrDev& pd = ctx->psrs[ctx->inst[k].psr].dev;
                const int ntr = (pd.red0c + 1 + pd.vns) / 16, ntc = pd.vkp / 16;
                const int nsk = ntr - (pd.red0c + 1 + 15) / 16;
                int t = pd.vb ? 1 : 0;
                for (int ti = 0; ti < ntr; ti++)
                    for (int tj = ti; tj < ntc; tj++)
                        if (!(ti >= ntr - nsk && (tj < ntr || pd.vb))) t++;
                return (long)(4 * t + pd.red0c + 1) * ctx->inst[k].n;
            };
            std::vector<long> ck(ninst, 0);
            for (auto& b : bucket) {
                for (int k : b) ck[k] = cost(k);
                std::stable_sort(b.begin(), b.end(), [&](int x, int y) { return ck[x] > ck[y]; });
                const int k1 = ncu / std::max(1, nsplit);
                const bool uniform = b.empty() || ck[b.front()] == ck[b.back()];
                if (ctx->gv_pair && !uniform && k1 > 0 && (int)b.size() > 2 * k1) {
                    std::vector<int> o(b.begin(), b.begin() + k1);
                    o.insert(o.end(), b.rbegin(), b.rbegin() + k1);
                    o.insert(o.end(), b.begin() + k1, b.end() - k1);
                    b.swap(o);
                }
            }
        }
        bool ident = true;
        int nxt = 0;
        for (int T = 0; T <= maxT; T++) {
            if (bucket[T].empty()) continue;
            KpGroup g{T, (int)sorted.size(), (int)bucket[T].size(), bkp[T]};
            for (int k : bucket[T]) {
                ident = ident && k == nxt++;
                sorted.push_back(ctx->inst[k]);
            }
            groups.push_back(g);
// ... 226 lines not shown
static void launch_resid2(pint_ctx* ctx, bool wt) {
    const size_t wlds = wt ? sizeof(double) * std::max((RES_BT / 64) * 32 * WT_CS2, 4 * 256) : 0;
    const double* ep = ctx->efz ? ctx->d_epart : nullptr;
    if (!ctx->efz && ctx->small && ctx->maxn <= RES_SMALLN)
        hipLaunchKernelGGL(k_resid2<64>, dim3((ctx->nrblk + 3) / 4), dim3(RES_BT), wlds, ctx->stream, ctx->d_psrs,
                           ctx->d_inst, ctx->d_rblk_inst, ctx->nrblk, ctx->d_ftay, ctx->d_rt, ctx->d_rp, ctx->d_rpart,
                           wt ? ctx->d_wtile : nullptr, ep);
    else
        hipLaunchKernelGGL(k_resid2<RES_BT>, dim3(ctx->nrblk), dim3(RES_BT), wlds, ctx->stream, ctx->d_psrs,
                           ctx->d_inst, ctx->d_rblk_inst, ctx->nrblk, ctx->d_ftay, ctx->d_rt, ctx->d_rp, ctx->d_rpart,
                           wt ? ctx->d_wtile : nullptr, ep);
}

static bool can_defer_r2(const pint_ctx* ctx) {
    return ctx->fuse_r2 && ctx->m_compact && ctx->n_vg == ctx->ninst && ctx->max_nep == 0 && !ctx->wbfit &&
           ctx->maxn <= 64 * (ctx->efz ? EF_ROWS : RES_RB);
}

static void flush_r2(pint_ctx* ctx) {
    if (!ctx->r2_pending) return;
    ctx->r2_pending = false;
    launch_resid2(ctx, false);
}

int pint_eval(pint_ctx* ctx, int want_M) {
    if (!ctx || ctx->ninst <= 0) return PINT_E_INVALID;
    hipSetDevice(ctx->device);
    if (want_M < 0 || want_M > 2) return PINT_E_INVALID;
    ctx->r2_pending = false;
    if (want_M) ctx->m_compact = (want_M == 2) ? 1 : 0;
    int write_red = 0;
    if (want_M) {
        write_red = ctx->red_valid[want_M == 2] ? 0 : 1;
        ctx->red_valid[want_M == 2] = 1;
        ctx->red_valid[want_M != 2] = 0;
        if (ctx->dm_noise_pend) {
            if (int rc = flush_cq_now(ctx)) return rc;
            HIPCHK(hipStreamWaitEvent(ctx->stream, ctx->ev_copied, 0));
            ctx->dm_noise_pend = false;
        }
    }
    record(ctx, want_M ? 2 : 0);
    const double* tabs = ctx->d_tables;
    const InstConst* icp = ctx->d_ic;
    EvalRestore rs{nullptr, nullptr, nullptr, nullptr, nullptr};
    if (!ctx->ic_valid) {
        if (ctx->restore_pending && ctx->ic0_valid) {
            tabs = ctx->d_tables0;
            icp = ctx->d_ic0;
            rs.tables = ctx->d_tables;
            rs.ic = ctx->d_ic;
        } else {
            launch_prep(ctx, ctx->d_tables, ctx->restore_pending ? (const double*)ctx->d_tables0 : nullptr, ctx->d_ic);
            HIPCHK(hipGetLastError());
        }
        ctx->restore_pending = false;
        ctx->ic_valid = true;
    }
    if (ctx->efz && ctx->nrblk > 0) {
        rs.rph = ctx->d_rp;
        rs.epart = ctx->d_epart;
    }
    const bool spin_pass = want_M && ctx->spin_grid && ctx->tables_fresh && ctx->spin_eval && rs.tables == nullptr &&
                           !ctx->efz && ctx->d_shr && ctx->blk_off[PINT_NBIN] == ctx->blk_off[1];
    if (ctx->d_swg) {
        hipLaunchKernelGGL(k_sw_geom, dim3(spin_pass ? 1 : ctx->ninst, (ctx->maxn + 256) / 256), dim3(256), 0, ctx->stream,
                           ctx->d_psrs, ctx->d_inst, icp, ctx->d_swg);
        HIPCHK(hipGetLastError());
        rs.swg = ctx->d_swg;
    }
    if (spin_pass) {
        const int n1 = ctx->inst[0].n + 1;
        hipLaunchKernelGGL(k_eval_head, dim3((n1 + 255) / 256), dim3(256), 0, ctx->stream, ctx->d_psrs, ctx->d_inst,
                           tabs, icp, rs.swg, ctx->d_shr);
        hipLaunchKernelGGL(k_eval_spin, dim3((ctx->ninst + 3) / 4), dim3(256), 0, ctx->stream, ctx->d_psrs, ctx->d_inst,
                           ctx->ninst, tabs, icp, ctx->d_shr, ctx->d_phhi, ctx->d_phlo, ctx->d_ftay, ctx->d_delay,
                           ctx->d_M);
        HIPCHK(hipGetLastError());
        ctx->n_spin_eval++;
    }
    int ntyp = 0;
    for (int t = 0; t < 3; t++) ntyp += ctx->blk_off[t + 1] > ctx->blk_off[t];
    const bool mix = ((ctx->eval_merge >> (want_M ? 1 : 0)) & 1) && (ntyp > 1 || (ctx->eval_merge & 4));
    if (!spin_pass && mix && ctx->nblk > 0) {
#define PINT_EVAL_MIX(WM)                                                                                      \
        hipLaunchKernelGGL((k_eval_mix<WM>), dim3(ctx->nblk), dim3(256), 0, ctx->stream, ctx->d_psrs, ctx->d_inst, \
                           ctx->d_blk_inst, ctx->d_blk_row0, ctx->blk_off[1], ctx->blk_off[2], ctx->blk_off[3],   \
                           tabs, icp, ctx->d_phhi, ctx->d_phlo, ctx->d_ftay, ctx->d_delay, ctx->d_M, \
                           ctx->d_dmxv, want_M == 2 ? 1 : 0, write_red, ctx->d_status, ctx->d_istatus, ctx->d_dfac, rs)
        const bool small = ctx->nblk <= 2 * 256;
        if (want_M && ctx->eval_wpe == 3 && !small) {
            hipLaunchKernelGGL((k_eval_mix_w<1, 3>), dim3(ctx->nblk), dim3(256), 0, ctx->stream, ctx->d_psrs, ctx->d_inst,
                               ctx->d_blk_inst, ctx->d_blk_row0, ctx->blk_off[1], ctx->blk_off[2], ctx->blk_off[3],
                               tabs, icp, ctx->d_phhi, ctx->d_phlo, ctx->d_ftay, ctx->d_delay, ctx->d_M,
                               ctx->d_dmxv, want_M == 2 ? 1 : 0, write_red, ctx->d_status, ctx->d_istatus, ctx->d_dfac, rs);
        } else if (want_M && ctx->eval_wpe == 4) {
            hipLaunchKernelGGL((k_eval_mix_w<1, 4>), dim3(ctx->nblk), dim3(256), 0, ctx->stream, ctx->d_psrs, ctx->d_inst,
                               ctx->d_blk_inst, ctx->d_blk_row0, ctx->blk_off[1], ctx->blk_off[2], ctx->blk_off[3],
                               tabs, icp, ctx->d_phhi, ctx->d_phlo, ctx->d_ftay, ctx->d_delay, ctx->d_M,
                               ctx->d_dmxv, want_M == 2 ? 1 : 0, write_red, ctx->d_status, ctx->d_istatus, ctx->d_dfac, rs);
        } else if (want_M) PINT_EVAL_MIX(1); else PINT_EVAL_MIX(0);
#undef PINT_EVAL_MIX
        HIPCHK(hipGetLastError());
    }
    for (int t = spin_pass ? PINT_NBIN : (mix ? 3 : 0); t < PINT_NBIN; t++) {
        int nb = ctx->blk_off[t + 1] - ctx->blk_off[t];
        if (nb == 0) continue;
        const int* bi = ctx->d_blk_inst + ctx->blk_off[t];
        const int* br = ctx->d_blk_row0 + ctx->blk_off[t];
#define PINT_EVAL_LAUNCH(WM, BT, ...)                                                                     \
        hipLaunchKernelGGL((k_eval<WM, BT, ##__VA_ARGS__>), dim3(nb), dim3(256), 0, ctx->stream, ctx->d_psrs, ctx->d_inst, bi, br, \
                           tabs, icp, ctx->d_phhi, ctx->d_phlo, ctx->d_ftay, ctx->d_delay, ctx->d_M, \
                           ctx->d_dmxv, want_M == 2 ? 1 : 0, write_red, ctx->d_status, ctx->d_istatus, ctx->d_dfac, rs)
        if (t == 0 && ctx->eval0_wpe) {
            if (want_M) PINT_EVAL_LAUNCH(1, 0, 6); else PINT_EVAL_LAUNCH(0, 0, 8);
        } else if (want_M && (t == 1 || t == 2) && ctx->evalb_wpe == 3 && nb > 2 * 256) {
            if (t == 1) PINT_EVAL_LAUNCH(1, 1, 3); else PINT_EVAL_LAUNCH(1, 2, 3);
        } else if (want_M) {
            switch (t) {
                case 0: PINT_EVAL_LAUNCH(1, 0); break;
                case 1: PINT_EVAL_LAUNCH(1, 1); break;
                case 2: PINT_EVAL_LAUNCH(1, 2); break;
                case 3: PINT_EVAL_LAUNCH(1, 3); break;
                case 4: PINT_EVAL_LAUNCH(1, 4); break;
                default: PINT_EVAL_LAUNCH(1, 5); break;
            }
        } else {
            switch (t) {
                case 0: PINT_EVAL_LAUNCH(0, 0); break;
                case 1: PINT_EVAL_LAUNCH(0, 1); break;
                case 2: PINT_EVAL_LAUNCH(0, 2); break;
                case 3: PINT_EVAL_LAUNCH(0, 3); break;
                case 4: PINT_EVAL_LAUNCH(0, 4); break;
                default: PINT_EVAL_LAUNCH(0, 5); break;
            }
        }
#undef PINT_EVAL_LAUNCH
        HIPCHK(hipGetLastError());
    }
    if (ctx->any_wavex) {
        auto kw = ctx->any_chrom ? k_wavex<true> : k_wavex<false>;
        hipLaunchKernelGGL(kw, dim3(ctx->ninst, (ctx->maxn + 256) / 256), dim3(256), 0, ctx->stream, ctx->d_psrs,
                           ctx->d_inst, tabs, icp, ctx->d_delay, ctx->d_phhi, ctx->d_phlo, want_M ? ctx->d_M : nullptr,
                           want_M == 2 ? 1 : 0, ctx->d_status, ctx->d_istatus);
        HIPCHK(hipGetLastError());
    }
    if (ctx->any_glitch) {
        hipLaunchKernelGGL(k_glitch, dim3(ctx->ninst, (ctx->maxn + 256) / 256), dim3(256), 0, ctx->stream, ctx->d_psrs,
                           ctx->d_inst, tabs, icp, ctx->d_delay, ctx->d_phhi, ctx->d_phlo, want_M ? ctx->d_M : nullptr,
                           want_M == 2 ? 1 : 0);
        HIPCHK(hipGetLastError());
    }
    record(ctx, want_M ? 3 : 1);
    record(ctx, 4);
    if (ctx->nrblk > 0) {
        const bool wt = ctx->wfuse && want_M == 0;
        const bool defer2 = want_M == 2 && can_defer_r2(ctx);
        const bool fused12 = !ctx->efz && ctx->small && ctx->maxn <= RES_SMALLN && !wt && !defer2 && ctx->resid12;
        if (ctx->efz) {
        } else if (fused12) {
            hipLaunchKernelGGL(k_resid12, dim3((ctx->nrblk + 3) / 4), dim3(RES_BT), 0, ctx->stream, ctx->d_psrs,
                               ctx->d_inst, ctx->d_rblk_inst, ctx->nrblk, ctx->d_phhi, ctx->d_phlo, ctx->d_ftay,
                               ctx->d_rt, ctx->d_rp, ctx->d_rpart);
        } else if (ctx->small && ctx->maxn <= RES_SMALLN) {
            const int nb4 = (ctx->nrblk + 3) / 4;
            hipLaunchKernelGGL(k_resid1<64>, dim3(nb4), dim3(RES_BT), 0, ctx->stream, ctx->d_psrs, ctx->d_inst,
                               ctx->d_rblk_inst, ctx->nrblk, ctx->d_phhi, ctx->d_phlo, ctx->d_rp, ctx->d_rpart);
        } else {
            hipLaunchKernelGGL(k_resid1<RES_BT>, dim3(ctx->nrblk), dim3(RES_BT), 0, ctx->stream, ctx->d_psrs,
                               ctx->d_inst, ctx->d_rblk_inst, ctx->nrblk, ctx->d_phhi, ctx->d_phlo, ctx->d_rp,
                               ctx->d_rpart);
        }
        if (defer2) ctx->r2_pending = true;
        else if (!fused12) launch_resid2(ctx, wt);
        ctx->chi2_pending = true;
        ctx->wtile_valid = wt;
    }
    HIPCHK(hipGetLastError());
    record(ctx, 5);
    if (ctx->lazy) return PINT_OK;
    int rc = check_status(ctx);
    update_timings(ctx);
    return rc;
}

int pint_read_resids(pint_ctx* ctx, double* time_resid, double* phase_resid, double* chi2) {
    flush_r2(ctx);
    if (chi2 && ctx->chi2_pending) {
        hipLaunchKernelGGL(k_rsum, dim3(ctx->ninst), dim3(64), 0, ctx->stream, ctx->d_inst, ctx->d_rpart, ctx->d_chi2);
        HIPCHK(hipGetLastError());
        ctx->chi2_pending = false;
    }
    if (time_resid) HIPCHK(d2h(time_resid, ctx->d_rt, sizeof(double) * ctx->tot_out, ctx->stream));
    if (phase_resid) HIPCHK(d2h(phase_resid, ctx->d_rp, sizeof(double) * ctx->tot_out, ctx->stream));
    if (chi2) HIPCHK(d2h(chi2, ctx->d_chi2, sizeof(double) * ctx->ninst, ctx->stream));
    if (!ctx->lazy) HIPCHK(hipStreamSynchronize(ctx->stream));
    return PINT_OK;
}

int pint_set_wideband(pint_ctx* ctx, int psr, const double* pp_dm, const double* pp_dme, const double* dm_sigma,
                      const uint64_t* dmjump_mask) {
    if (!ctx || psr < 0 || psr >= (int)ctx->psrs.size() || !pp_dm || !pp_dme || !dm_sigma) return PINT_E_INVALID;
    hipSetDevice(ctx->device);
    if (int rc_ = commit_uploads(ctx)) return rc_;
    PsrHost& ph = ctx->psrs[psr];
    if (ph.spec.ndmjump > 0 && !dmjump_mask) { ctx->err = "DMJUMPs without masks"; return PINT_E_INVALID; }
    if (ph.dev.nwx + ph.dev.ndmwx > 0) {
        ctx->err = "wideband DM data with WaveX / DMWaveX is not supported";
        return PINT_E_INVALID;
    }
    if (ph.dev.ncm + ph.dev.ncmwx > 0) {
        ctx->err = "wideband DM data with ChromaticCM / CMWaveX is not supported";
        return PINT_E_INVALID;
    }
    for (int i = 0; i < ph.n; i++)
// ... 618 lines not shown
    return PINT_OK;
}

int pint_chi2_gls(pint_ctx* ctx, double* chi2) {
    flush_r2(ctx);
    if (flush_chi2(ctx)) return PINT_E_HIP;
    int R = 0;
    for (int pi : ctx->upsr) R = 2 * ctx->psrs[pi].spec.nred > R ? 2 * ctx->psrs[pi].spec.nred : R;
    int stride = R + 2;
    int nsw = ctx->nsplit;
    if (ctx->wtile_valid) {
        nsw = 1;
        stride = ctx->wstride;
    }
    size_t need = (size_t)ctx->ninst * nsw * stride;
    if (need > ctx->wpart_cap) {
        if (ctx->capturing) { ctx->err = "pint_chi2_gls: first call inside a graph capture"; return PINT_E_INVALID; }
        dfree((void*&)ctx->d_wpart);
        HIPCHK(cmalloc((void**)&ctx->d_wpart, sizeof(double) * need));
        ctx->wpart_cap = need;
    }
    record(ctx, 10);
    if (ctx->sigma_pending) HIPCHK(hipStreamWaitEvent(ctx->stream, ctx->ev_sigma, 0));
    if (!ctx->wtile_valid) {
        hipLaunchKernelGGL(k_wdot, dim3(nsw, ctx->ninst), dim3(256), 0, ctx->stream, ctx->d_psrs, ctx->d_inst, ctx->d_M,
                           ctx->d_rt, nsw, stride, ctx->m_compact, ctx->d_wpart);
        HIPCHK(hipGetLastError());
    }
    hipLaunchKernelGGL(k_wsolve, dim3(ctx->ninst), dim3(256), sizeof(double) * ((R + 1) + (R + 1) * (R + 2) / 2),
                       ctx->stream, ctx->d_psrs,
                       ctx->d_inst, ctx->d_rt, ctx->d_sigL, ctx->d_esum, ctx->d_eD, ctx->d_eW, ctx->d_wpart, nsw,
                       stride, ctx->d_ecs, ctx->d_chi2g, ctx->d_lognorm,
                       ctx->wtile_valid ? (const double*)ctx->d_wtile : nullptr, (const double*)ctx->d_rpart,
                       ctx->d_chi2, ctx->m_compact);
    HIPCHK(hipGetLastError());
    if (ctx->wtile_valid) ctx->chi2_pending = false;
    record(ctx, 11);
    if (ctx->lazy && !ctx->capturing) {
        ctx->chi2_dst = chi2;
        return PINT_OK;
    }
    HIPCHK(d2h(chi2, ctx->d_chi2g, sizeof(double) * ctx->ninst, ctx->stream));
    if (!ctx->lazy) HIPCHK(hipStreamSynchronize(ctx->stream));
    return PINT_OK;
}

int pint_chi2_wls(pint_ctx* ctx, double* chi2) {
    if (!ctx || ctx->ninst <= 0 || !chi2) return PINT_E_INVALID;
    flush_r2(ctx);
    if (flush_chi2(ctx)) return PINT_E_HIP;
    hipSetDevice(ctx->device);
    hipLaunchKernelGGL(k_chi2w, dim3(ctx->ninst), dim3(256), 0, ctx->stream, ctx->d_psrs, ctx->d_inst, ctx->d_rt,
                       ctx->d_chi2g);
    HIPCHK(hipGetLastError());
    HIPCHK(d2h(chi2, ctx->d_chi2g, sizeof(double) * ctx->ninst, ctx->stream));
    if (!ctx->lazy) HIPCHK(hipStreamSynchronize(ctx->stream));
    return PINT_OK;
}

int pint_set_lazy(pint_ctx* ctx, int lazy) {
    ctx->lazy = lazy;
    return PINT_OK;
}

int pint_set_option(pint_ctx* ctx, int key, int value) {
    if (!ctx) return PINT_E_INVALID;
    if (key == PINT_OPT_BLOCKED_SOLVE) { ctx->blocked_solve = value ? 1 : 0; return PINT_OK; }
    if (key == PINT_OPT_VGRAM) { ctx->vgram = value ? 1 : 0; return PINT_OK; }
    if (key == PINT_OPT_VBIN) { ctx->vbin = value ? 1 : 0; return PINT_OK; }
    if (key == PINT_OPT_WBFIT) { ctx->wbfit = value ? 1 : 0; return PINT_OK; }
    if (key == PINT_OPT_COV_DEFER) {
        if (value < 0 || value > 2) return PINT_E_INVALID;
        ctx->cov_defer = value;
        return PINT_OK;
    }
    if (key == PINT_OPT_REFINE) { ctx->refine = value ? 1 : 0; return PINT_OK; }
    if (key == PINT_OPT_SCHUR) { ctx->schur = value ? 1 : 0; return PINT_OK; }
    if (key == PINT_OPT_SMALL) { ctx->small = value ? 1 : 0; return PINT_OK; }
    if (key == PINT_OPT_LA_CHOL) { ctx->la_chol = value ? 1 : 0; return PINT_OK; }
    if (key == PINT_OPT_SOLVE_W8) { ctx->solve_w8 = value ? 1 : 0; return PINT_OK; }
    if (key == PINT_OPT_EFUSE) { ctx->efuse = value ? 1 : 0; return PINT_OK; }
    if (key == PINT_OPT_LANE_SOLVE) { ctx->lane_solve = value ? 1 : 0; return PINT_OK; }
    if (key == PINT_OPT_SPIN_EVAL) { ctx->spin_eval = value ? 1 : 0; return PINT_OK; }
    if (key == PINT_OPT_TIMING_EVERY) {
        if (value < 1) return PINT_E_INVALID;
        ctx->timing_every = value;
        ctx->gram_calls = 0;
        return PINT_OK;
    }
    if (key == 99) { ctx->gvdbg = value; return PINT_OK; }
    if (key == PINT_OPT_TIMING_MASK) {
        ctx->timing_mask = value & 0xff;
        for (int sl = 0; sl < pint_ctx::NSLOT; sl++)
            for (int k = 0; k < pint_ctx::NEV; k++) ctx->rec_slot[sl][k] = false;
        for (int k = 0; k < pint_ctx::NMS; k++) ctx->ms[k] = 0.0f;
        return PINT_OK;
    }
    ctx->err = "unknown option";
    return PINT_E_INVALID;
}

static void join_side_streams(pint_ctx* ctx) {
    if (ctx->sigma_pending) hipStreamWaitEvent(ctx->stream, ctx->ev_sigma, 0);
    if (any_copy_pend(ctx)) hipStreamWaitEvent(ctx->stream, ctx->ev_copied, 0);
    ctx->sigma_pending = false;
    clear_copy_pend(ctx);
}

int pint_capture_begin(pint_ctx* ctx) {
    if (!ctx || ctx->ninst <= 0 || ctx->capturing) return PINT_E_INVALID;
    if (!ctx->lazy) { ctx->err = "graph capture needs lazy mode"; return PINT_E_INVALID; }
    hipSetDevice(ctx->device);
    if (int rc = flush_cq_now(ctx)) return rc;
    HIPCHK(hipStreamSynchronize(ctx->cstream));
    HIPCHK(hipStreamSynchronize(ctx->sstream));
    HIPCHK(hipStreamSynchronize(ctx->stream));
    ctx->sigma_pending = false;
    clear_copy_pend(ctx);
    HIPCHK(hipStreamBeginCapture(ctx->stream, hipStreamCaptureModeRelaxed));
    ctx->capturing = true;
    return PINT_OK;
}

int pint_capture_end(pint_ctx* ctx) {
    if (!ctx || !ctx->capturing) return PINT_E_INVALID;
    join_side_streams(ctx);
    ctx->capturing = false;
    hipGraph_t g = nullptr;
    HIPCHK(hipStreamEndCapture(ctx->stream, &g));
    const int s = ctx->slot;
    if (ctx->graph_exec_s[s]) hipGraphExecDestroy(ctx->graph_exec_s[s]);
    if (ctx->graph_s[s]) hipGraphDestroy(ctx->graph_s[s]);
    ctx->graph_s[s] = g;
    ctx->graph_exec_s[s] = nullptr;
    HIPCHK(hipGraphInstantiate(&ctx->graph_exec_s[s], g, nullptr, nullptr, 0));
    return PINT_OK;
}

int pint_graph_launch(pint_ctx* ctx) {
    if (!ctx || !ctx->graph_exec_s[ctx->slot]) {
        if (ctx) ctx->err = "pint_graph_launch: no graph captured for this pipeline slot";
        return PINT_E_INVALID;
    }
    hipSetDevice(ctx->device);
    join_side_streams(ctx);
    HIPCHK(hipGraphLaunch(ctx->graph_exec_s[ctx->slot], ctx->stream));
    return PINT_OK;
}

int pint_lognorm(pint_ctx* ctx, int gls, double* out) {
    if (!ctx || ctx->ninst <= 0 || !out) return PINT_E_INVALID;
    if (gls == 2) {
        for (int k = 0; k < ctx->ninst; k++) {
            const PsrDev& d = ctx->psrs[ctx->inst[k].psr].dev;
            out[k] = ctx->psrs[ctx->inst[k].psr].spec.wb_noones
                         ? d.logsig
                         : 0.5 * (2.0 * d.logsig + std::log(1e40) + std::log(1e-40 + d.sumw));
        }
    } else if (gls) {
        HIPCHK(d2h(out, ctx->d_lognorm, sizeof(double) * ctx->ninst, ctx->stream));
        HIPCHK(hipStreamSynchronize(ctx->stream));
    } else {
        for (int k = 0; k < ctx->ninst; k++) out[k] = ctx->psrs[ctx->inst[k].psr].dev.logsig;
    }
    return PINT_OK;
}
// ... 80 lines not shown
    if ((dpars || errs || cov || chi2lin) && (rc = pint_read_step(ctx, dpars, errs, cov, chi2lin))) return rc;
    lap("read_step");
    if ((noise_red || noise_ecorr) && (rc = pint_noise_resids(ctx, noise_red, noise_ecorr))) return rc;
    if (noise_dm && (rc = pint_noise_resids_dm(ctx, noise_dm))) return rc;
    lap("noise");
    if ((rc = pint_eval(ctx, 0))) return rc;
    lap("eval");
    if (chi2 && (rc = pint_chi2_gls(ctx, chi2))) return rc;
    lap("chi2_gls");
    rc = pint_step_end(ctx, slot);
    lap("step_end");
    return rc;
}

int pint_check_step(pint_ctx* ctx, int s) {
    if (!ctx || s < 0 || s >= pint_ctx::NSLOT) return PINT_E_INVALID;
    hipSetDevice(ctx->device);
    HIPCHK(hipEventSynchronize(ctx->ev_done[s]));
    if (ctx->cdone_rec[s]) HIPCHK(hipEventSynchronize(ctx->ev_cdone[s]));
    ctx->cdone_rec[s] = false;
    ctx->copy_pend[s] = false;
    const int st = ctx->h_status[s];
    if (st) {
        ctx->h_status[s] = 0;
        HIPCHK(hipMemsetAsync(ctx->d_status_slots + s, 0, sizeof(int), ctx->stream));
    }
    hipEvent_t* ev = ctx->ev;
    bool* rec = ctx->rec;
    ctx->ev = ctx->ev_slot[s];
    ctx->rec = ctx->rec_slot[s];
    update_timings(ctx, true);
    for (int k = 0; k < pint_ctx::NEV; k++) ctx->rec[k] = false;
    ctx->ev = ev;
    ctx->rec = rec;
    return decode_status(ctx, st);
}

int pint_last_timing(pint_ctx* ctx, double* ms) {
    update_timings(ctx);
    for (int k = 0; k < pint_ctx::NMS; k++) ms[k] = ctx->ms[k];
    return PINT_OK;
}

int pint_debug_read(pint_ctx* ctx, int which, double* out) {
    HIPCHK(hipStreamSynchronize(ctx->sstream));
    if (which == 5) {
        static unsigned long long t[4096 * 5];
        HIPCHK(hipStreamSynchronize(ctx->stream));
        HIPCHK(hipMemcpyFromSymbol(t, HIP_SYMBOL(g_gvts), sizeof(t)));
        for (int i = 0; i < 4096 * 5; i++) out[i] = (double)t[i];
        return 4096;
    }
    if (which == 4) {
        unsigned long long ts[32];
        HIPCHK(hipStreamSynchronize(ctx->stream));
        HIPCHK(hipMemcpyFromSymbol(ts, HIP_SYMBOL(g_ts), sizeof(ts)));
        for (int i = 0; i < 32; i++) out[i] = (double)(long long)(ts[i] - ts[0]) * 0.01;
        return 32;
    }
    if (which == 7) {
        static unsigned long long t[WGT_K * WGT_B * 2];
        HIPCHK(hipStreamSynchronize(ctx->stream));
        HIPCHK(hipMemcpyFromSymbol(t, HIP_SYMBOL(g_wgt), sizeof(t)));
        for (int i = 0; i < WGT_K * WGT_B * 2; i++) out[i] = (double)t[i];
        return WGT_K * WGT_B * 2;
    }
    if (which == 9) {
        static unsigned long long t[WGT_B * 2];
        HIPCHK(hipStreamSynchronize(ctx->stream));
        HIPCHK(hipMemcpyFromSymbol(t, HIP_SYMBOL(g_wgp), sizeof(t)));
        for (int i = 0; i < WGT_B * 2; i++) out[i] = (double)t[i];
        return WGT_B * 2;
    }
    if (which == 8) {
        static unsigned long long z[WGT_K * WGT_B * 2];
        HIPCHK(hipStreamSynchronize(ctx->stream));
        HIPCHK(hipMemcpyToSymbol(HIP_SYMBOL(g_wgt), z, sizeof(z)));
        HIPCHK(hipMemcpyToSymbol(HIP_SYMBOL(g_wgp), z, sizeof(unsigned long long) * WGT_B * 2));
        const int on = out && out[0] != 0.0 ? 1 : 0;
        HIPCHK(hipMemcpyToSymbol(HIP_SYMBOL(g_wgt_on), &on, sizeof(on)));
        HIPCHK(hipDeviceSynchronize());
        return on;
    }
    if (which == 6) {
        unsigned long long z[32] = {0};
        HIPCHK(hipStreamSynchronize(ctx->stream));
        HIPCHK(hipMemcpyToSymbol(HIP_SYMBOL(g_ts), z, sizeof(z)));
        return 32;
    }
    size_t n = which == 0 ? ctx->tot_g : which == 1 ? ctx->tot_c * ctx->nsplit : ctx->tot_s;
    double* src = which == 0 ? ctx->d_G : which == 1 ? ctx->d_colsq : which == 2 ? ctx->d_sigL : ctx->d_work;
    HIPCHK(d2h(out, src, sizeof(double) * n, ctx->stream));
    HIPCHK(hipStreamSynchronize(ctx->stream));
    return ctx->nsplit;
}

int pint_inst_status(pint_ctx* ctx, int32_t* out) {
    if (!ctx || ctx->ninst <= 0 || !out) return PINT_E_INVALID;
    hipSetDevice(ctx->device);
    HIPCHK(d2h(out, ctx->d_istatus, sizeof(int) * ctx->ninst, ctx->stream));
    HIPCHK(hipMemsetAsync(ctx->d_istatus, 0, sizeof(int) * ctx->ninst, ctx->stream));
    HIPCHK(hipStreamSynchronize(ctx->stream));
    return PINT_OK;
}

int pint_noise_resids(pint_ctx* ctx, double* red, double* ecorr) {
    if (!ctx || ctx->ninst <= 0) return PINT_E_INVALID;
    hipSetDevice(ctx->device);
    const long need = 3 * std::max<long>(1, ctx->tot_out);
    if (need > ctx->noise_cap) {
        if (ctx->capturing) { ctx->err = "pint_noise_resids: first call inside a graph capture"; return PINT_E_INVALID; }
        dfree((void*&)ctx->d_noise);
        HIPCHK(cmalloc((void**)&ctx->d_noise, sizeof(double) * need));
        ctx->noise_cap = need;
    }
    double* dr = ctx->d_noise;
    double* de = ctx->d_noise + std::max<long>(1, ctx->tot_out);
    int maxn = 1;
    for (auto& I : ctx->inst) maxn = std::max(maxn, I.n);
    if (ctx->lazy && !ctx->capturing) {
        const int ninst = ctx->ninst, maxep = ctx->max_nep, cmp = ctx->m_compact;
        const long tot = ctx->tot_out;
        const double* d_dp = ctx->d_dpars;
        const PsrDev* psrs = ctx->d_psrs;
        const InstDev* insts = ctx->d_inst;
        double *d_es = ctx->d_esum, *d_eD = ctx->d_eD, *d_eC = ctx->d_eC, *d_df = ctx->d_dfac;
        ctx->cq.push_back([=]() -> int {
            hipStream_t st = ctx->cstream;
            HostLap lap{"noise op"};
            if (red)
                hipLaunchKernelGGL(k_noise_red, dim3((maxn + 255) / 256, ninst), dim3(256), 0, st, psrs, insts, d_dp, dr, 0,
                                   d_df);
            if (ecorr) {
                HIPCHK(hipMemsetAsync(de, 0, sizeof(double) * tot, st));
                if (maxep > 0)
                    hipLaunchKernelGGL(k_noise_ecorr, dim3(maxep, ninst), dim3(64), 0, st, psrs, insts, d_dp, d_es, d_eD,
                                       de, cmp, d_eC);
            }
            HIPCHK(hipGetLastError());
            lap("kernels");
            if (red)
                if (int rc = export_seg(ctx, red, dr, tot)) return rc;
            if (ecorr)
                if (int rc = export_seg(ctx, ecorr, de, tot)) return rc;
            return PINT_OK;
        });
        return PINT_OK;
    }
    hipStream_t st = ctx->stream;
    if (ctx->lazy) {
        st = ctx->cstream;
        HIPCHK(hipStreamWaitEvent(st, ctx->ev_solved, 0));
    }
    if (red)
        hipLaunchKernelGGL(k_noise_red, dim3((maxn + 255) / 256, ctx->ninst), dim3(256), 0, st, ctx->d_psrs,
                           ctx->d_inst, ctx->d_dpars, dr, 0, ctx->d_dfac);
    if (ecorr) {
        HIPCHK(hipMemsetAsync(de, 0, sizeof(double) * ctx->tot_out, st));
        if (ctx->max_nep > 0)
            hipLaunchKernelGGL(k_noise_ecorr, dim3(ctx->max_nep, ctx->ninst), dim3(64), 0, st, ctx->d_psrs,
                               ctx->d_inst, ctx->d_dpars, ctx->d_esum, ctx->d_eD, de, ctx->m_compact, ctx->d_eC);
    }
    if (hipGetLastError() != hipSuccess) { ctx->err = "pint_noise_resids: launch failed"; return PINT_E_HIP; }
    if (red) HIPCHK(d2h(red, dr, sizeof(double) * ctx->tot_out, st));
    if (ecorr) HIPCHK(d2h(ecorr, de, sizeof(double) * ctx->tot_out, st));
    if (ctx->lazy) {
// ... 244 lines not shown
```

pint_amd/engine.py:

```python
from __future__ import annotations

import ctypes as C
import os
from dataclasses import dataclass, field
from typing import Dict, List, Optional, Sequence

import numpy as np

from . import _lib as L
from .noise import red_noise_freqs_weights, scaled_sigma_us
from .parameter import LD
from .timing_model import BIN_IDS, GLITCH_PROPS, OBLIQUITY, TimingModel

UNITS = {
    "RAJ": "1 / (hourangle Hz)", "DECJ": "1 / (deg Hz)", "ELONG": "1 / (deg Hz)", "ELAT": "1 / (deg Hz)",
}


def split_ld(v) -> tuple:
    v = LD(v)
    hi = float(v)
    lo = float(v - LD(hi))
    return hi, lo

# ... 738 lines not shown
        try:
            out = fn()
        except Exception:
            self.L.pint_capture_end(self.ctx)
            raise
        self._check(self.L.pint_capture_end(self.ctx))
        return out

    def replay(self):
        self._check(self.L.pint_graph_launch(self.ctx))

    def set_tables(self, tabs):
        tabs = np.asarray(tabs, dtype=np.float64).ravel()
        if self.lazy and "tables" not in self._inflight:
            buf = self._pin("tables", tabs.size)
            buf[:] = tabs
            tabs = buf
            self._inflight.add("tables")
        else:
            tabs = np.array(tabs, dtype=np.float64)
            self._keep.append(tabs)
        self._check(self.L.pint_set_tables(self.ctx, L.ptr(tabs)))

    def _split(self, flat, sizes):
        out, o = [], 0
        for s in sizes:
            out.append(flat[o:o + s])
            o += s
        return out

    def read_resids(self):
        n = [l.n for l in self.inst_layout]
        tr = np.empty(sum(n))
        pr = np.empty(sum(n))
        c2 = np.empty(len(n))
        self._check(self.L.pint_read_resids(self.ctx, L.ptr(tr), L.ptr(pr), L.ptr(c2)))
        return self._split(tr, n), self._split(pr, n), c2

    def set_wideband(self, lay):
        from .noise import scaled_dm_sigma
        model, toas = lay.model, lay.toas
        try:
            dm, dme = toas.get_dms(), toas.get_dm_errors()
        except AttributeError:
            raise ValueError("Input TOA object does not have wideband DM values")
        if len(dm) != lay.n or len(dme) != lay.n:
            raise ValueError("Input TOA object' DM data and DM errors do not match.")
        sig = scaled_dm_sigma(model, toas)
        jm = np.zeros(lay.n, dtype=np.uint64)
        for k, name in enumerate(model.mask_params("DMJUMP")):
            p = model[name]
            jm[toas.select_mask(p.key, p.key_value)] |= np.uint64(1) << np.uint64(k)
        dm, dme = np.ascontiguousarray(dm, dtype=np.float64), np.ascontiguousarray(dme, dtype=np.float64)
        self._check(self.L.pint_set_wideband(self.ctx, lay.psr_id, L.ptr(dm), L.ptr(dme), L.ptr(sig),
                                             L.ptr(jm, C.c_uint64)))
        lay.keep += [dm, dme, sig, jm]
        lay.dm_data, lay.dm_error, lay.dm_sigma = dm, dme, sig

    def dm_resids(self, subtract_mean=False, use_weighted_mean=True):
        n = [l.n for l in self.inst_layout]
        r = np.empty(sum(n))
        c2 = np.empty(len(n))
        self._check(self.L.pint_dm_resids(self.ctx, 1 if subtract_mean else 0, 1 if use_weighted_mean else 0,
                                          L.ptr(r), L.ptr(c2)))
        return self._split(r, n), c2

    def read_chi2(self):
        c2 = self._pin("chi2r", len(self.inst_layout))
        self._check(self.L.pint_read_resids(self.ctx, None, None, L.ptr(c2)))
        return c2 if self.lazy else c2.copy()

    def read_eval(self):
        rows = [l.n + 1 for l in self.inst_layout]
        a = [np.empty(sum(rows)) for _ in range(4)]
        self._check(self.L.pint_read_eval(self.ctx, *[L.ptr(x) for x in a]))
        return [self._split(x, rows) for x in a]

    def read_designmatrix(self):
        sizes = [l.n * l.K for l in self.inst_layout]
        M = np.empty(sum(sizes))
        self._check(self.L.pint_read_designmatrix(self.ctx, L.ptr(M)))
        return [m.reshape(l.K, l.n).T for m, l in zip(self._split(M, sizes), self.inst_layout)]

    def set_lazy(self, lazy=True):
        self._check(self.L.pint_set_lazy(self.ctx, 1 if lazy else 0))
        self.lazy = bool(lazy)

    def fit_layout(self, lay):
        out = np.zeros(4, dtype=np.int32)
        self._check(self.L.pint_fit_layout(self.ctx, lay.psr_id, L.ptr(out, C.c_int32)))
        return tuple(int(x) for x in out)

    def vgram_layout(self, lay):
        out = np.zeros(4, dtype=np.int32)
        self._check(self.L.pint_vgram_layout(self.ctx, lay.psr_id, L.ptr(out, C.c_int32)))
        return tuple(int(x) for x in out)

    def set_blocked_solve(self, on=True):
        self._check(self.L.pint_set_option(self.ctx, 1, 1 if on else 0))

    def set_timing_mask(self, mask=0xFF):
        self._check(self.L.pint_set_option(self.ctx, 3, int(mask)))

    def set_timing_every(self, k=1):
        self._check(self.L.pint_set_option(self.ctx, 8, int(k)))

    def set_refine(self, on=True):
        self._check(self.L.pint_set_option(self.ctx, 4, 1 if on else 0))

    def set_vgram(self, on=True):
        self._check(self.L.pint_set_option(self.ctx, 2, 1 if on else 0))

    def set_wbfit(self, on=True):
        self._check(self.L.pint_set_option(self.ctx, 6, 1 if on else 0))

    def set_cov_defer(self, mode=1):
        self._check(self.L.pint_set_option(self.ctx, 7, int(mode)))

    def set_schur(self, on=True):
        self._check(self.L.pint_set_option(self.ctx, 9, 1 if on else 0))

    def set_small(self, on=True):
        self._check(self.L.pint_set_option(self.ctx, 10, 1 if on else 0))

    def set_la_chol(self, on=True):
        self._check(self.L.pint_set_option(self.ctx, 11, 1 if on else 0))

    def set_efuse(self, on=True):
        self._check(self.L.pint_set_option(self.ctx, 12, 1 if on else 0))

    def set_lane_solve(self, on=True):
        self._check(self.L.pint_set_option(self.ctx, 13, 1 if on else 0))

    def set_spin_eval(self, on=True):
        self._check(self.L.pint_set_option(self.ctx, 14, 1 if on else 0))

    def set_solve_w8(self, on=True):
        self._check(self.L.pint_set_option(self.ctx, 15, 1 if on else 0))

    def set_vbin(self, on=True):
        self._check(self.L.pint_set_option(self.ctx, 5, 1 if on else 0))

    def n_vgram(self):
        return int(self.L.pint_query(self.ctx, 1))

    def n_spin_eval(self):
        return int(self.L.pint_query(self.ctx, 3))

    def nsplit(self):
        return int(self.L.pint_query(self.ctx, 2))

    def check(self):
        try:
            self._check(self.L.pint_check(self.ctx))
        finally:
            self._inflight.clear()
            self._keep.clear()

    def step_end(self) -> int:
        sl = C.c_int(-1)
        self._check(self.L.pint_step_end(self.ctx, C.byref(sl)))
        self._closed(sl.value)
        return sl.value

    def _closed(self, sl):
        self._slot_state[sl] = (self._inflight, self._keep)
        self._pending.add(sl)
        self._slot = (sl + 1) % L.NSLOT
        self._inflight, self._keep = self._slot_state[self._slot]

    def fit_step_enqueue(self, restore=True, lam=1.0, want_cov=True, noise=True):
        if not self.lazy:
            raise RuntimeError("fit_step_enqueue needs lazy mode (set_lazy(True))")
        lays = self.inst_layout
        ok = self._off_k
        dp, er = self._pin("dp", ok[-1]), self._pin("er", ok[-1])
        cov = self._pin("cov", self._off_cov[-1]) if want_cov else None
        cl = self._pin("cl", len(ok) - 1)
        n = int(self._off_n[-1])
        red = ec = dm = None
        if noise:
            if any(l.spec.dmn0 > 0 for l in lays):
                red = self._pin("noise_red", n)
            if any("EcorrNoise" in l.model.components for l in lays):
                ec = self._pin("noise_ec", n)
            if any(l.spec.dmn0 < l.nred for l in lays):
                dm = self._pin("noise_dm", n)
        c2 = self._pin("chi2g", len(lays))
        sl = C.c_int(-1)
        self._check(self.L.pint_fit_step_enqueue(self.ctx, 1 if restore else 0, 1, float(lam), L.ptr(dp), L.ptr(er),
                                                 L.ptr(cov), L.ptr(cl), L.ptr(red), L.ptr(ec), L.ptr(dm), L.ptr(c2),
                                                 C.byref(sl)))
        self._closed(sl.value)
        covs = SplitView(cov, self._off_cov, self._cov_shapes) if want_cov else []
        nz = _NoiseViews(lays, self._off_n, red, ec, dm) if noise else None
        return sl.value, (SplitView(dp, ok), SplitView(er, ok), covs, cl), nz, c2

    def check_step(self, slot: int):
        rc = self.L.pint_check_step(self.ctx, int(slot))
        self._pending.discard(int(slot))
        inflight, keep = self._slot_state[slot]
        inflight.clear()
        keep.clear()
        self._check(rc)

    def read_step(self, want_cov=True):
        ok = self._off_k
        get = self._pin if self.lazy else (lambda name, n: np.empty(max(1, int(n))))
        dp = get("dp", ok[-1])
        er = get("er", ok[-1])
        cov = get("cov", self._off_cov[-1]) if want_cov else None
        cl = get("cl", len(ok) - 1)
        self._check(self.L.pint_read_step(self.ctx, L.ptr(dp), L.ptr(er), L.ptr(cov), L.ptr(cl)))
        covs = SplitView(cov, self._off_cov, self._cov_shapes) if want_cov else []
        return SplitView(dp, ok), SplitView(er, ok), covs, cl

    def read_tables(self):
        return self._split(self.read_tables_flat(), [l.tstride for l in self.inst_layout])

    def read_tables_flat(self):
        t = np.empty(self.ntab)
# ... 246 lines not shown
```

Baseline: 207,500 fits/s.

## Specialize eval kernels to LDS-staged params with uniform run loads and global-space reads

Adds a GEN template flag so the default eval path assumes parameter tables and column runs are always staged in LDS, removing the per-thread runtime choice between LDS and global pointers. When any instance exceeds the staging limits, or the new option is off, a single merged generic kernel dispatches by block offset across the binary models. It also forces column-run fields to be wave-uniform via readfirstlane so they can live in scalar registers, and casts TOA loads to the global address space to avoid flat-address loads. This adds another kernel variant and extra template instantiations, which may raise code size and register pressure.

```diff
diff --git a/include/pint_amd.h b/include/pint_amd.h
--- a/include/pint_amd.h
+++ b/include/pint_amd.h
@@ -206,6 +206,7 @@
 #define PINT_OPT_LANE_SOLVE 13
 #define PINT_OPT_SPIN_EVAL 14
 #define PINT_OPT_SOLVE_W8 15
+#define PINT_OPT_EVAL_LDS 16
 int pint_set_option(pint_ctx *ctx, int key, int value);
 #define PINT_EIG_MAXDEG 8
 int pint_solve_eig(pint_ctx *ctx, int mode, const double *threshold, int32_t *ndeg, double *degvec,
diff --git a/pint_amd/csrc/physics.hpp b/pint_amd/csrc/physics.hpp
--- a/pint_amd/csrc/physics.hpp
+++ b/pint_amd/csrc/physics.hpp
@@ -33,6 +33,23 @@
 __device__ __constant__ const double INV_LO[NINV] = {0.0, 0.0, 0.0, 1.850371707708594e-17, 0.0, -1.1102230246251566e-17, 9.25185853854297e-18, 7.93016446160826e-18, 0.0, 6.1679056923619804e-18, -5.551115123125783e-18, -2.523234146875356e-18, 4.625929269271485e-18, -4.270088556250602e-18, 3.96508223080413e-18, 9.251858538542971e-19, 0.0, 8.163404592832033e-19, 3.0839528461809902e-18, 2.921639538487254e-18, -2.7755575615628915e-18, 2.64338815386942e-18, -1.261617073437678e-18, 1.206764157201257e-18, 2.3129646346357427e-18, -8.326672684688674e-19, -2.135044278125301e-18, 2.05596856412066e-18, 1.982541115402065e-18, 4.785444071660157e-19, 4.625929269271486e-19, 8.953411488912552e-19, 0.0, -8.410780489584519e-19, 4.0817022964160166e-19, 8.921435019309293e-19, 1.5419764230904951e-18, -1.50030138462859e-18, 1.460819769243627e-18, 8.896017825522087e-19, -1.3877787807814458e-18, -8.46206573647223e-19, 1.32169407693471e-18, 3.2273925134452225e-19, -6.30808536718839e-19, -8.480870326997723e-19, 6.033820786006285e-19, 5.167261417803255e-19, 1.1564823173178713e-18, 1.6285159162231251e-18, -4.163336342344337e-19, 2.7211348642773444e-19, -1.0675221390626506e-18, 7.20073895688486e-19, 1.02798428206033e-18, 8.831319514063744e-19, 9.912705577010326e-19, 9.73879846162418e-19, 2.3927220358300787e-19, 5.880418562633244e-20, 2.312964634635743e-19, -8.531426931033477e-19, 4.476705744456276e-19, 8.8112938462314e-19};
 PD double inv_int(int k) { return k < NINV ? INV_HI[k] : 1.0 / (double)k; }
 PD dd dd_div_int(dd a, int k) { return k < NINV ? dd_mul(a, dd_make(INV_HI[k], INV_LO[k])) : dd_div_d(a, (double)k); }
+
+PD int uni(int v) {
+#if defined(__HIP_DEVICE_COMPILE__)
+    return __builtin_amdgcn_readfirstlane(v);
+#else
+    return v;
+#endif
+}
+
+template <class T>
+PD T gld(const T* p, long i) {
+#if defined(__HIP_DEVICE_COMPILE__)
+    return ((const __attribute__((address_space(1))) T*)p)[i];
+#else
+    return p[i];
+#endif
+}
 
 PD double pval(const double* P, int o) { return P[o] + P[o + 1]; }
 PD dd pdd(const double* P, int o) { return dd_make(P[o], P[o + 1]); }
@@ -964,6 +981,10 @@
     int dcol0;
     int pad_[3];
 };
+PD ColRun run_uni(const ColRun* runs, int u) {
+    const ColRun R = runs[u];
+    return ColRun{uni(R.kind), uni(R.col0), uni(R.cnt), uni(R.idx0), uni(R.dcol0), {0, 0, 0}};
+}
 
 struct EvalHead {
     double delay;
@@ -1034,7 +1055,7 @@
 PD void glitch_row_columns(const pint_spec_t& S, const double* P, dd tdb, double delay, double iF0, double* Mb,
                            unsigned r, long ld, const ColRun* runs, int nrun, bool compact) {
     for (int u = 0; u < nrun; u++) {
-        const ColRun R = runs[u];
+        const ColRun R = run_uni(runs, u);
         if (R.kind != PINT_COL_GLITCH) continue;
         double* colp = Mb + (long)(compact ? R.dcol0 : R.col0) * ld;
         for (int j = 0; j < R.cnt; j++, colp += ld) {
@@ -1069,7 +1090,7 @@
     const double dmc = chain * DMCONST * h.inv_f2;
     o.dmc = dmc;
     for (int u = 0; u < nrun; u++) {
-        const ColRun R = runs[u];
+        const ColRun R = run_uni(runs, u);
         if (compact && R.kind == PINT_COL_DMX) continue;
         double* colp = Mb + (long)(compact ? R.dcol0 : R.col0) * ld;
         switch (R.kind) {
@@ -1103,7 +1124,7 @@
                 if (swg) {
                     unsigned rr = r;
                     asm volatile("" : "+v"(rr));
-                    g = swg[rr];
+                    g = gld(swg, rr);
                 }
                 colp[r] = h.inv_f2 > 1.0 ? 0.0 : dmc * g;
             } break;
@@ -1111,7 +1132,7 @@
                 for (int j = 0; j < R.cnt; j++, colp += ld) {
                     const int idx = R.idx0 + j;
                     bool in = t.dmx_a == idx || t.dmx_b == idx;
-                    for (int k = t.dmx_x0; k < t.dmx_x1; k++) in |= t.dmx_x[k] == idx;
+                    for (int k = t.dmx_x0; k < t.dmx_x1; k++) in |= gld(t.dmx_x, k) == idx;
                     colp[r] = in ? dmc : 0.0;
                 }
                 break;
@@ -1168,7 +1189,7 @@
         if (S.shapiro == 2) {
 #pragma unroll 1
             for (int q = 0; q < 5; q++) {
-                const double x = t.planet[3 * q], y = t.planet[3 * q + 1], z = t.planet[3 * q + 2];
+                const double x = gld(t.planet, 3 * q), y = gld(t.planet, 3 * q + 1), z = gld(t.planet, 3 * q + 2);
                 const double rp = sqrt(x * x + y * y + z * z);
                 const double rcp = x * L[0] + y * L[1] + z * L[2];
                 ds += -2.0 * TPLANET[q] * log((rp - rcp) * INV_AU_KM);
@@ -1183,7 +1204,7 @@
     }
     double inv_f2 = 1.0 / (bfreq * bfreq);
     o.inv_f2 = inv_f2;
-    if (S.o_NE_SW >= 0) delay += (pval(P, S.o_NE_SW) * swg[r]) * DMCONST * inv_f2;
+    if (S.o_NE_SW >= 0) delay += (pval(P, S.o_NE_SW) * gld(swg, r)) * DMCONST * inv_f2;
     double dt_yr_dm = 0.0;
     if (S.ndm > 0) {
         bool any = false;
@@ -1201,7 +1222,7 @@
         double dmx = 0.0;
         if (t.dmx_a >= 0) dmx += pval(P, S.o_DMX + 2 * t.dmx_a);
         if (t.dmx_b >= 0) dmx += pval(P, S.o_DMX + 2 * t.dmx_b);
-        for (int k = t.dmx_x0; k < t.dmx_x1; k++) dmx += pval(P, S.o_DMX + 2 * t.dmx_x[k]);
+        for (int k = t.dmx_x0; k < t.dmx_x1; k++) dmx += pval(P, S.o_DMX + 2 * gld(t.dmx_x, k));
         delay += dmx * DMCONST * inv_f2;
     }
     double logf = 0.0;
@@ -1245,7 +1266,7 @@
     EvalPre pre;
     eval_pre(S, P, C, t, o, true, pre, swg, r);
     h = pre.h;
-    if (S.o_NE_SW >= 0) h.swg = swg[r];
+    if (S.o_NE_SW >= 0) h.swg = gld(swg, r);
     if (S.nfd > 0) h.delay += pre.fd;
 }
 
@@ -1290,11 +1311,11 @@
         Ell1Grad eg;
         if (BIN == 1 || BIN == 3) ell1_grad<BIN == 3>(B, eg);
         for (int u = 0; u < nrun; u++) {
-            const ColRun R = runs[u];
+            const ColRun R = run_uni(runs, u);
             if (R.kind != PINT_COL_BIN) continue;
             double* colp = Mb + (long)(compact ? R.dcol0 : R.col0) * ld;
             for (int j = 0; j < R.cnt; j++, colp += ld) {
-                const int pid = S.col_index[R.col0 + j];
+                const int pid = uni(S.col_index[R.col0 + j]);
                 double d = 0.0;
                 if (BIN == 1 || BIN == 3) d = ell1_deriv(B, eg, pid);
                 if (BIN == 2) d = ddm_deriv(B, pid);
diff --git a/pint_amd/csrc/pint_hip.hip b/pint_amd/csrc/pint_hip.hip
--- a/pint_amd/csrc/pint_hip.hip
+++ b/pint_amd/csrc/pint_hip.hip
@@ -360,25 +360,25 @@
 };
 
 __device__ __forceinline__ void load_toa_row(const PsrDev& Pd, const pint_spec_t& S, unsigned r, ToaRow& t) {
-    t.tdb = dd_make(Pd.tdb_hi[r], Pd.tdb_lo[r]);
-    t.freq = Pd.freq[r];
+    t.tdb = dd_make(gld(Pd.tdb_hi, r), gld(Pd.tdb_lo, r));
+    t.freq = gld(Pd.freq, r);
 #pragma unroll
     for (int k = 0; k < 3; k++) {
-        t.pos[k] = Pd.pos[3 * r + k];
-        t.vel[k] = Pd.vel[3 * r + k];
-        t.sun[k] = Pd.sun[3 * r + k];
+        t.pos[k] = gld(Pd.pos, 3 * r + k);
+        t.vel[k] = gld(Pd.vel, 3 * r + k);
+        t.sun[k] = gld(Pd.sun, 3 * r + k);
     }
     t.planet = S.shapiro == 2 ? Pd.planet + 15 * r : nullptr;
-    t.flags = Pd.flags[r];
-    t.jmask = Pd.jmask[r];
-    t.dmx_a = Pd.dmx_a[r];
-    t.dmx_b = Pd.dmx_b[r];
+    t.flags = gld(Pd.flags, r);
+    t.jmask = gld(Pd.jmask, r);
+    t.dmx_a = gld(Pd.dmx_a, r);
+    t.dmx_b = gld(Pd.dmx_b, r);
     t.dmx_x = Pd.dmx_x;
-    t.dmx_x0 = Pd.dmx_x ? Pd.dmx_x[r] : 0;
-    t.dmx_x1 = Pd.dmx_x ? Pd.dmx_x[r + 1] : 0;
-}
-
-template <int WANT_M, int BIN>
+    t.dmx_x0 = Pd.dmx_x ? gld(Pd.dmx_x, r) : 0;
+    t.dmx_x1 = Pd.dmx_x ? gld(Pd.dmx_x, r + 1) : 0;
+}
+
+template <int WANT_M, int BIN, bool GEN>
 __device__ __forceinline__ void eval_row(const pint_spec_t& S, EvalLds& L, const PsrDev& Pd, const InstDev& I, bool stP,
                                          bool stR, int nrun, const double* __restrict__ tables, unsigned r, int n,
                                          bool own, double* __restrict__ Mout, double* __restrict__ dmxv, int compact,
@@ -386,13 +386,16 @@
                                          double* __restrict__ ph_hi, double* __restrict__ ph_lo,
                                          double* __restrict__ ftay, double* __restrict__ delay_out,
                                          double* __restrict__ dfac, const double* __restrict__ swg, EvalOut& o) {
-    const double* P = stP ? L.P : tables + I.toff;
     ToaRow t;
     load_toa_row(Pd, S, r, t);
     double* Mb = WANT_M ? (Mout + I.moff) : nullptr;
     const bool rowM = WANT_M && own && r < (unsigned)n;
     const bool cmp = WANT_M && compact && Pd.dsplit;
-    eval_toa<BIN>(S, P, L.C, t, o, rowM ? Mb : nullptr, r, n, stR ? L.R : Pd.runs, nrun, cmp, swg ? swg + I.roff : nullptr);
+    if (GEN)
+        eval_toa<BIN>(S, stP ? L.P : tables + I.toff, L.C, t, o, rowM ? Mb : nullptr, r, n, stR ? L.R : Pd.runs, nrun, cmp,
+                      swg ? swg + I.roff : nullptr);
+    else
+        eval_toa<BIN>(S, L.P, L.C, t, o, rowM ? Mb : nullptr, r, n, L.R, nrun, cmp, swg ? swg + I.roff : nullptr);
     if (!own) return;
     if (rowM && cmp) dmxv[I.ooff + r] = o.dmc;
     if (o.status) {
@@ -410,7 +413,7 @@
         dd ts = dd_mul_d(t.tdb, DAYSEC);
         double* colp = Mb + (long)(cmp ? Pd.red0c : S.ncol) * n;
         for (int k = write_red ? 0 : S.dmn0; k < S.nred; k++) {
-            dd x = dd_mul(ts, dd_make(Pd.red_freq[k], Pd.red_freq[S.nred + k]));
+            dd x = dd_mul(ts, dd_make(gld(Pd.red_freq, k), gld(Pd.red_freq, S.nred + k)));
             double fr = dd_to_d(dd_sub(x, dd_floor(x)));
             double sn, cs;
             sincos(TWO_PI * fr, &sn, &cs);
@@ -421,7 +424,7 @@
     }
 }
 
-template <int WANT_M, int BIN>
+template <int WANT_M, int BIN, bool GEN = false>
 __device__ __forceinline__ void eval_block(int b, const PsrDev* __restrict__ psrs, const InstDev* __restrict__ insts,
                                            const int* __restrict__ blk_inst, const int* __restrict__ blk_row0,
                                            const double* __restrict__ tables, const InstConst* __restrict__ ic,
@@ -434,7 +437,7 @@
     const InstDev I = insts[ii];
     const PsrDev& Pd = psrs[I.psr];
     const int ts = I.ts, nrun = I.nrun;
-    const bool stP = ts <= EVAL_MAXTAB, stR = nrun <= EVAL_MAXRUN;
+    const bool stP = !GEN || ts <= EVAL_MAXTAB, stR = !GEN || nrun <= EVAL_MAXRUN;
     {
         static_assert(sizeof(pint_spec_t) % 16 == 0 && sizeof(InstConst) % 16 == 0 && sizeof(ColRun) % 16 == 0,
                       "eval staging: 16-byte words");
@@ -443,25 +446,26 @@
         static_assert(NS <= 512 && NC + EVAL_MAXRUN * RW <= 256 && EVAL_MAXTAB <= 512, "eval staging: two rounds of 256");
         const int t = threadIdx.x;
         const int NR = stR ? nrun * RW : 0;
-        const uint4* sg = reinterpret_cast<const uint4*>(I.spec);
-        const uint4* cg = reinterpret_cast<const uint4*>(ic + ii);
-        const uint4* rg = reinterpret_cast<const uint4*>(I.runs);
+        typedef unsigned int w16 __attribute__((ext_vector_type(4)));
+        const w16* sg = reinterpret_cast<const w16*>(I.spec);
+        const w16* cg = reinterpret_cast<const w16*>(ic + ii);
+        const w16* rg = reinterpret_cast<const w16*>(I.runs);
         const double* pg = tables + I.toff;
         const bool hs0 = t < NS, hs1 = t + 256 < NS, hc = t < NC, hr = !hc && t < NC + NR;
         const bool hp0 = stP && t < ts, hp1 = stP && t + 256 < ts;
-        uint4 s0 = {}, s1 = {}, cr = {};
+        w16 s0 = 0, s1 = 0, cr = 0;
         double p0 = 0.0, p1 = 0.0;
-        if (hs0) s0 = sg[t];
-        if (hs1) s1 = sg[t + 256];
+        if (hs0) s0 = gld(sg, t);
+        if (hs1) s1 = gld(sg, t + 256);
         if (hc) cr = cg[t];
-        else if (hr) cr = rg[t - NC];
+        else if (hr) cr = gld(rg, t - NC);
         if (hp0) p0 = pg[t];
         if (hp1) p1 = pg[t + 256];
-        uint4* sd = reinterpret_cast<uint4*>(&L.S);
+        w16* sd = reinterpret_cast<w16*>(&L.S);
         if (hs0) sd[t] = s0;
         if (hs1) sd[t + 256] = s1;
-        if (hc) reinterpret_cast<uint4*>(&L.C)[t] = cr;
-        else if (hr) reinterpret_cast<uint4*>(L.R)[t - NC] = cr;
+        if (hc) reinterpret_cast<w16*>(&L.C)[t] = cr;
+        else if (hr) reinterpret_cast<w16*>(L.R)[t - NC] = cr;
         if (hp0) L.P[t] = p0;
         if (hp1) L.P[t + 256] = p1;
     }
@@ -489,7 +493,7 @@
         if (!own) return;
     }
     EvalOut o;
-    eval_row<WANT_M, BIN>(S, L, Pd, I, stP, stR, nrun, tables, r, n, own, Mout, dmxv, compact, write_red, status, istatus,
+    eval_row<WANT_M, BIN, GEN>(S, L, Pd, I, stP, stR, nrun, tables, r, n, own, Mout, dmxv, compact, write_red, status, istatus,
                           ii, ph_hi, ph_lo, ftay, delay_out, dfac, rs.swg, o);
     wgp_stamp(1, false);
     if (!ef) return;
@@ -503,19 +507,19 @@
     __syncthreads();
     const dd tz = dd_make(L.X[0], L.X[1]);
     dd d0 = dd_make(0.0);
-    if (!S.track_pn && S.subtract_mean) d0 = dd_add_d(dd_sub(dd_make(L.X[2], L.X[3]), tz), Pd.dpn[0]);
+    if (!S.track_pn && S.subtract_mean) d0 = dd_add_d(dd_sub(dd_make(L.X[2], L.X[3]), tz), gld(Pd.dpn, 0));
     double sw = 0.0, swx = 0.0;
     if (lt < EF_ROWS && own) {
-        const dd d = dd_add_d(dd_sub(dd_make(o.phase.hi, o.phase.lo), tz), Pd.dpn[r]);
+        const dd d = dd_add_d(dd_sub(dd_make(o.phase.hi, o.phase.lo), tz), gld(Pd.dpn, r));
         double full;
         if (S.track_pn) {
-            full = dd_to_d(dd_add_d(d, -Pd.pn[r]));
+            full = dd_to_d(dd_add_d(d, -gld(Pd.pn, r)));
         } else {
             const dd x = dd_sub(d, d0);
             full = dd_to_d(dd_sub(x, dd_round_half_up(x)));
         }
         rs.rph[I.roff - ii + r] = full;
-        const double lw = Pd.isig[r];
+        const double lw = gld(Pd.isig, r);
         const double w = S.weighted_mean ? lw * lw : 1.0;
         sw += w;
         swx += w * full;
@@ -751,13 +755,13 @@
     double* Mb = Mout + I.moff;
     for (int r = threadIdx.x & 63; r <= n; r += 64) {
         ToaRow t;
-        t.tdb = dd_make(Pd.tdb_hi[r], Pd.tdb_lo[r]);
-        t.jmask = Pd.jmask[r];
-        t.dmx_a = Pd.dmx_a[r];
-        t.dmx_b = Pd.dmx_b[r];
+        t.tdb = dd_make(gld(Pd.tdb_hi, r), gld(Pd.tdb_lo, r));
+        t.jmask = gld(Pd.jmask, r);
+        t.dmx_a = gld(Pd.dmx_a, r);
+        t.dmx_b = gld(Pd.dmx_b, r);
         t.dmx_x = Pd.dmx_x;
-        t.dmx_x0 = Pd.dmx_x ? Pd.dmx_x[r] : 0;
-        t.dmx_x1 = Pd.dmx_x ? Pd.dmx_x[r + 1] : 0;
+        t.dmx_x0 = Pd.dmx_x ? gld(Pd.dmx_x, r) : 0;
+        t.dmx_x1 = Pd.dmx_x ? gld(Pd.dmx_x, r + 1) : 0;
         const double* q = shr + (long)r * EVAL_HEAD_W;
         const EvalHead h = {q[0], q[1], q[2], q[3], q[4], q[5], q[6], q[7], q[8], q[9]};
         EvalOut o;
@@ -774,7 +778,7 @@
     }
 }
 
-template <int WANT_M, int BIN, int W = 0>
+template <int WANT_M, int BIN, int W = 0, bool GEN = false>
 __global__ __launch_bounds__(256) __attribute__((amdgpu_waves_per_eu(W > 0 ? W : 1, W > 0 ? W : 10)))
 void k_eval(const PsrDev* __restrict__ psrs, const InstDev* __restrict__ insts,
                                               const int* __restrict__ blk_inst, const int* __restrict__ blk_row0,
@@ -785,7 +789,7 @@
                                               int write_red, int* __restrict__ status, int* __restrict__ istatus,
                                               double* __restrict__ dfac, EvalRestore rs) {
     __shared__ EvalLds L;
-    eval_block<WANT_M, BIN>(blockIdx.x, psrs, insts, blk_inst, blk_row0, tables, ic, ph_hi, ph_lo, ftay, delay_out,
+    eval_block<WANT_M, BIN, GEN>(blockIdx.x, psrs, insts, blk_inst, blk_row0, tables, ic, ph_hi, ph_lo, ftay, delay_out,
                             Mout, dmxv, compact, write_red, status, istatus, dfac, L, rs);
 }
 
@@ -831,6 +835,34 @@
 __global__ __launch_bounds__(256) __attribute__((amdgpu_waves_per_eu(W, W))) void k_eval_mix_w(PINT_EVAL_MIX_ARGS) {
     WgTimer wgt_(WGT_EVAL);
     eval_mix_body<WANT_M>(PINT_EVAL_MIX_PASS);
+}
+
+struct EvalOffs {
+    int v[PINT_NBIN + 1];
+};
+template <int WANT_M>
+__global__ __launch_bounds__(256) void k_eval_gen(const PsrDev* __restrict__ psrs, const InstDev* __restrict__ insts,
+                                                  const int* __restrict__ blk_inst, const int* __restrict__ blk_row0,
+                                                  EvalOffs off, const double* __restrict__ tables,
+                                                  const InstConst* __restrict__ ic, double* __restrict__ ph_hi,
+                                                  double* __restrict__ ph_lo, double* __restrict__ ftay,
+                                                  double* __restrict__ delay_out, double* __restrict__ Mout,
+                                                  double* __restrict__ dmxv, int compact, int write_red,
+                                                  int* __restrict__ status, int* __restrict__ istatus,
+                                                  double* __restrict__ dfac, EvalRestore rs) {
+    static_assert(PINT_NBIN == 6, "k_eval_gen: one case per binary model");
+    const int b = blockIdx.x;
+    __shared__ EvalLds L;
+#define PINT_EVAL_GEN(BT)                                                                                         \
+    eval_block<WANT_M, BT, true>(b, psrs, insts, blk_inst, blk_row0, tables, ic, ph_hi, ph_lo, ftay, delay_out, Mout, \
+                                 dmxv, compact, write_red, status, istatus, dfac, L, rs)
+    if (b < off.v[1]) PINT_EVAL_GEN(0);
+    else if (b < off.v[2]) PINT_EVAL_GEN(1);
+    else if (b < off.v[3]) PINT_EVAL_GEN(2);
+    else if (b < off.v[4]) PINT_EVAL_GEN(3);
+    else if (b < off.v[5]) PINT_EVAL_GEN(4);
+    else PINT_EVAL_GEN(5);
+#undef PINT_EVAL_GEN
 }
 
 constexpr int RES_BT = 256;
@@ -4967,6 +4999,8 @@
     int solve_w8 = 1;
     int eval0_wpe = 1;
     int eval_wpe = 3;
+    int eval_lds = 1;
+    bool eval_staged = true;
     int n_vg = 0;
     bool any_dmx_rows = false;
     double *d_TSp = nullptr, *d_TS = nullptr;
@@ -5537,6 +5571,7 @@
     ctx->efuse = getenv("PINT_EFUSE") ? atoi(getenv("PINT_EFUSE")) : 1;
     ctx->lane_solve = getenv("PINT_LANE_SOLVE") ? atoi(getenv("PINT_LANE_SOLVE")) : 1;
     ctx->spin_eval = getenv("PINT_SPIN_EVAL") ? atoi(getenv("PINT_SPIN_EVAL")) : 1;
+    ctx->eval_lds = getenv("PINT_EVAL_LDS") ? (atoi(getenv("PINT_EVAL_LDS")) ? 1 : 0) : 1;
     hipEventCreateWithFlags(&ctx->ev_gram, evf);
     hipEventCreateWithFlags(&ctx->ev_sigma, evf);
     for (int sl = 0; sl < pint_ctx::NSLOT; sl++) {
@@ -6461,9 +6496,11 @@
     ctx->maxK = maxK;
     ctx->maxn = 0;
     ctx->max_ts = 0;
+    ctx->eval_staged = true;
     for (const InstDev& I : ctx->inst) {
         ctx->maxn = std::max(ctx->maxn, I.n);
         ctx->max_ts = std::max(ctx->max_ts, ctx->psrs[I.psr].spec.tstride);
+        if (I.ts > EVAL_MAXTAB || I.nrun > EVAL_MAXRUN) ctx->eval_staged = false;
     }
     {
         std::vector<char> seen(ctx->psrs.size(), 0);
@@ -6856,8 +6893,19 @@
     int ntyp = 0;
     for (int t = 0; t < 3; t++) ntyp += ctx->blk_off[t + 1] > ctx->blk_off[t];
     const bool mix = ((ctx->eval_merge >> (want_M ? 1 : 0)) & 1) && (ntyp > 1 || (ctx->eval_merge & 4));
-    if (!spin_pass && mix && ctx->nblk > 0) {
-#define PINT_EVAL_MIX(WM)                                                                                      \
+    const bool gen = !spin_pass && (!ctx->eval_lds || !ctx->eval_staged);
+    if (gen && ctx->blk_off[PINT_NBIN] > 0) {
+        EvalOffs off;
+        for (int t = 0; t <= PINT_NBIN; t++) off.v[t] = ctx->blk_off[t];
+        auto kg = want_M ? k_eval_gen<1> : k_eval_gen<0>;
+        hipLaunchKernelGGL(kg, dim3(ctx->blk_off[PINT_NBIN]), dim3(256), 0, ctx->stream, ctx->d_psrs, ctx->d_inst,
+                           ctx->d_blk_inst, ctx->d_blk_row0, off, tabs, icp, ctx->d_phhi, ctx->d_phlo, ctx->d_ftay,
+                           ctx->d_delay, ctx->d_M, ctx->d_dmxv, want_M == 2 ? 1 : 0, write_red, ctx->d_status,
+                           ctx->d_istatus, ctx->d_dfac, rs);
+        HIPCHK(hipGetLastError());
+    }
+    if (!spin_pass && !gen && mix && ctx->nblk > 0) {
+#define PINT_EVAL_MIX(WM)                                                                                     \
         hipLaunchKernelGGL((k_eval_mix<WM>), dim3(ctx->nblk), dim3(256), 0, ctx->stream, ctx->d_psrs, ctx->d_inst, \
                            ctx->d_blk_inst, ctx->d_blk_row0, ctx->blk_off[1], ctx->blk_off[2], ctx->blk_off[3],   \
                            tabs, icp, ctx->d_phhi, ctx->d_phlo, ctx->d_ftay, ctx->d_delay, ctx->d_M, \
@@ -6877,7 +6925,7 @@
 #undef PINT_EVAL_MIX
         HIPCHK(hipGetLastError());
     }
-    for (int t = spin_pass ? PINT_NBIN : (mix ? 3 : 0); t < PINT_NBIN; t++) {
+    for (int t = spin_pass || gen ? PINT_NBIN : (mix ? 3 : 0); t < PINT_NBIN; t++) {
         int nb = ctx->blk_off[t + 1] - ctx->blk_off[t];
         if (nb == 0) continue;
         const int* bi = ctx->d_blk_inst + ctx->blk_off[t];
@@ -6889,7 +6937,7 @@
         if (t == 0 && ctx->eval0_wpe) {
             if (want_M) PINT_EVAL_LAUNCH(1, 0, 6); else PINT_EVAL_LAUNCH(0, 0, 8);
         } else if (want_M && (t == 1 || t == 2) && ctx->evalb_wpe == 3 && nb > 2 * 256) {
-            if (t == 1) PINT_EVAL_LAUNCH(1, 1, 3); else PINT_EVAL_LAUNCH(1, 2, 3);
+            if (t == 1) PINT_EVAL_LAUNCH(1, 1, 3, true); else PINT_EVAL_LAUNCH(1, 2, 3);
         } else if (want_M) {
             switch (t) {
                 case 0: PINT_EVAL_LAUNCH(1, 0); break;
@@ -6902,9 +6950,9 @@
         } else {
             switch (t) {
                 case 0: PINT_EVAL_LAUNCH(0, 0); break;
-                case 1: PINT_EVAL_LAUNCH(0, 1); break;
+                case 1: PINT_EVAL_LAUNCH(0, 1, 0, true); break;
                 case 2: PINT_EVAL_LAUNCH(0, 2); break;
-                case 3: PINT_EVAL_LAUNCH(0, 3); break;
+                case 3: PINT_EVAL_LAUNCH(0, 3, 0, true); break;
                 case 4: PINT_EVAL_LAUNCH(0, 4); break;
                 default: PINT_EVAL_LAUNCH(0, 5); break;
             }
@@ -7689,6 +7737,7 @@
     if (key == PINT_OPT_EFUSE) { ctx->efuse = value ? 1 : 0; return PINT_OK; }
     if (key == PINT_OPT_LANE_SOLVE) { ctx->lane_solve = value ? 1 : 0; return PINT_OK; }
     if (key == PINT_OPT_SPIN_EVAL) { ctx->spin_eval = value ? 1 : 0; return PINT_OK; }
+    if (key == PINT_OPT_EVAL_LDS) { ctx->eval_lds = value ? 1 : 0; return PINT_OK; }
     if (key == PINT_OPT_TIMING_EVERY) {
         if (value < 1) return PINT_E_INVALID;
         ctx->timing_every = value;
@@ -7935,6 +7984,11 @@
         HIPCHK(hipDeviceSynchronize());
         return on;
     }
+    if (which == 10) {
+        HIPCHK(d2h(out, ctx->d_dmxv, sizeof(double) * ctx->tot_out, ctx->stream));
+        HIPCHK(hipStreamSynchronize(ctx->stream));
+        return (int)ctx->tot_out;
+    }
     if (which == 6) {
         unsigned long long z[32] = {0};
         HIPCHK(hipStreamSynchronize(ctx->stream));
diff --git a/pint_amd/engine.py b/pint_amd/engine.py
--- a/pint_amd/engine.py
+++ b/pint_amd/engine.py
@@ -844,6 +844,12 @@
         self._check(self.L.pint_read_designmatrix(self.ctx, L.ptr(M)))
         return [m.reshape(l.K, l.n).T for m, l in zip(self._split(M, sizes), self.inst_layout)]
 
+    def read_dmx_values(self):
+        rows = [l.n for l in self.inst_layout]
+        v = np.empty(max(1, sum(rows)))
+        self._check(min(0, self.L.pint_debug_read(self.ctx, 10, L.ptr(v))))
+        return self._split(v[:sum(rows)], rows)
+
     def set_lazy(self, lazy=True):
         self._check(self.L.pint_set_lazy(self.ctx, 1 if lazy else 0))
         self.lazy = bool(lazy)
@@ -899,6 +905,9 @@
 
     def set_solve_w8(self, on=True):
         self._check(self.L.pint_set_option(self.ctx, 15, 1 if on else 0))
+
+    def set_eval_lds(self, on=True):
+        self._check(self.L.pint_set_option(self.ctx, 16, 1 if on else 0))
 
     def set_vbin(self, on=True):
         self._check(self.L.pint_set_option(self.ctx, 5, 1 if on else 0))
```

Result: no change. 207,500 fits/s (-0.0%).
